# mir-group/allegro

Hardware: NVIDIA B200
Metric: atom-steps/sec (energy+forces) (higher is better)
Workload: dtype f32

## Files before the change

### allegro_b200/_lib.py

```python
from __future__ import annotations

import ctypes as C
import os
from typing import Optional, Sequence

import torch

from . import build as _build

AB2_F64, AB2_F32, AB2_BF16 = 0, 1, 2
ACT_NONE, ACT_SILU, ACT_MUL_DSILU = 0, 1, 2
EPI_NONE, EPI_MUL_DSILU = 0, 1
MAX_SEG = 4

DTYPE_ENUM = {torch.float64: AB2_F64, torch.float32: AB2_F32, torch.bfloat16: AB2_BF16}
ACC_DTYPE = {torch.float64: torch.float64, torch.float32: torch.float32, torch.bfloat16: torch.float32}

_LIB: Optional[C.CDLL] = None

_vp, _i64, _i32, _dbl = C.c_void_p, C.c_int64, C.c_int, C.c_double

_SIGNATURES = {
    "ab2_version": ([], C.c_int),
    "ab2_device_ok": ([], C.c_int),
    "ab2_last_error": ([], C.c_char_p),
    "ab2_set_option": ([C.c_char_p, _i32], C.c_int),
    "ab2_op_scatter_env": ([_i32, _i64, _i64, _dbl, _vp, _vp, _vp, _vp], C.c_int),
    "ab2_op_contract": ([_i32, _i32, _i64, _i32, _i32, _i32, _i32, _i32, _vp, _vp, _vp, _vp, _vp, _vp, _vp], C.c_int),
    "ab2_op_gather_rows": ([_i32, _i64, _i64, _dbl, _vp, _vp, _vp, _vp], C.c_int),
    "ab2_op_contract_wgrad": ([_i32, _i64, _i32, _i32, _i32, _i32, _i32, _vp, _vp, _vp, _vp, _vp, _vp, _vp], C.c_int),
    "ab2_sh_fwd": ([_i32, _i32, _i64, _vp, _vp, _vp], C.c_int),
    "ab2_sh_bwd": ([_i32, _i32, _i64, _vp, _vp, _vp, _i32, _vp], C.c_int),
    "ab2_linear": ([_i32, _i64, _i32, _i32, _i32, _vp, _vp, _vp, _vp, _vp, _i32, _vp, _vp, _i32, _vp, _vp, _vp, _vp, _i32, _vp, _i64, _vp], C.c_int),
    "ab2_linear_packed_bytes": ([_i32, _i32, _i32], C.c_int64),
    "ab2_linear_pack": ([_i32, _i32, _i32, _vp, _vp, _vp], C.c_int),
    "ab2_env_sum": ([_i32, _i32, _i64, _i32, _vp, _vp, _vp, _i64, _dbl, _vp, _vp], C.c_int),
    "ab2_env_bwd": ([_i32, _i32, _i64, _i64, _i32, _vp, _vp, _vp, _vp, _i64, _vp, _dbl, _vp, _i64, _vp, _vp], C.c_int),
    "ab2_tp_fwd": ([_i32, _i32, _i64, _i64, _i32, _i32, _i32, _i32, _vp, _vp, _vp, _vp, _vp, _vp, _i32, _vp, _vp, _i64, _vp, _vp], C.c_int),
    "ab2_tp_bwd": ([_i32, _i32, _i64, _i64, _i32, _i32, _i32, _i32, _vp, _vp, _vp, _vp, _vp, _vp, _i32, _vp, _vp, _i64, _vp, _vp, _vp, _i64, _vp, _vp, _vp], C.c_int),
    "ab2_edge_sum": ([_i32, _i64, _vp, _vp, _dbl, _vp, _vp], C.c_int),
    "ab2_edge_sum_bwd": ([_i32, _i64, _vp, _vp, _dbl, _vp, _vp], C.c_int),
    "ab2_force_scatter": ([_i32, _i64, _i64, _i64, _vp, _vp, _vp, _vp, _vp, _vp], C.c_int),
    "ab2_transpose_ui": ([_i32, _i64, _i32, _i32, _vp, _vp, _i32, _vp], C.c_int),
    "ab2_edge_vec": ([_i32, _i32, _i64, _vp, _vp, _vp, _vp, _vp, _vp], C.c_int),
    "ab2_radial_fwd": ([_i32, _i64, _i32, _i32, _dbl, _vp, _vp, _vp, _vp, _vp, _i32, _vp, _vp, _vp, _vp, _vp, _vp], C.c_int),
    "ab2_radial_pq_fwd": ([_i32, _i64, _i32, _i32, _dbl, _vp, _vp, _vp, _vp, _vp, _i32, _vp, _vp, _vp, _vp], C.c_int),
    "ab2_radial_pq_bwd": ([_i32, _i64, _i32, _i32, _dbl, _vp, _vp, _vp, _vp, _vp, _i32, _vp, _vp, _vp, _vp, _vp, _vp], C.c_int),
    "ab2_zbl": ([_i32, _i64, _i32, _dbl, _dbl, _vp, _vp, _vp, _vp, _vp, _vp, _vp, _vp, _vp], C.c_int),
    "ab2_p2p_mailbox_bytes": ([_i32, _i32], C.c_int64),
    "ab2_p2p_alloc": ([_i64, C.POINTER(C.c_void_p)], C.c_int),
    "ab2_p2p_free": ([_vp], C.c_int),
    "ab2_p2p_get_handle": ([_vp, _vp], C.c_int),
    "ab2_p2p_open_handle": ([_vp, C.POINTER(C.c_void_p)], C.c_int),
    "ab2_p2p_close_handle": ([_vp], C.c_int),
    "ab2_p2p_error": ([_vp, _i32, _i32, _vp], C.c_int),
    "ab2_p2p_begin": ([_vp, _vp], C.c_int),
    "ab2_p2p_push_rows": ([_i32, _i32, _i32, _vp, _vp, _i32, _dbl, _vp, _i32, _i32, _vp, _vp, _vp], C.c_int),
    "ab2_p2p_wait_unpack": ([_i32, _i32, _i32, _vp, _i32, _i32, _vp, _i32, _vp, _vp, _i32, _vp], C.c_int),
    "ab2_p2p_allreduce_energy": ([_vp, _i32, _i32, _i32, _vp, _vp, _vp, _vp, _vp], C.c_int),
    "ab2_nl_bin": ([_i32, _i64, _vp, _vp, _vp, _vp, _vp, _dbl, _vp, _vp], C.c_int),
    "ab2_nl_count": ([_i32, _i64, _vp, _vp, _vp, _vp, _vp, _dbl, _vp, _vp, _vp, _vp], C.c_int),
    "ab2_nl_fill": ([_i32, _i64, _vp, _vp, _vp, _vp, _vp, _dbl, _vp, _vp, _vp, _vp, _vp, _vp], C.c_int),
    "ab2_radial_bwd": ([_i32, _i64, _i32, _i32, _dbl, _vp, _vp, _vp, _vp, _vp, _i32, _vp, _vp, _vp, _vp, _vp, _vp, _vp], C.c_int),
}


def exported_symbols() -> Sequence[str]:
    return tuple(_SIGNATURES)


def lib_path() -> str:
    return _build.LIB


def load() -> C.CDLL:
    global _LIB
    if _LIB is not None:
        return _LIB
    path = lib_path()
    if not os.path.exists(path):
        if os.environ.get("ALLEGRO_B200_AUTOBUILD", "0") == "1":
            _build.build()
        else:
            raise RuntimeError(
                f"allegro_b200: CUDA extension {path} not built. Run `python -m allegro_b200.build` "
                "(or __graft_entry__.build()).  There is no CPU fallback."
            )
    lib = C.CDLL(path)
    for name, (args, res) in _SIGNATURES.items():
        fn = getattr(lib, name)
        fn.argtypes = args
        fn.restype = res
    _LIB = lib
    for kv in filter(None, os.environ.get("ALLEGRO_B200_OPTIONS", "").split(",")):
        k, v = kv.split("=")
        if lib.ab2_set_option(k.strip().encode(), int(v)) != 0:
            raise RuntimeError(f"ALLEGRO_B200_OPTIONS: unknown option {k!r}")
    return lib


class _Prof:

    def __init__(self):
        self.launches = 0
        self.enabled = False
        self.records = {}

    def reset(self):
        self.launches = 0
        self.records = {}

    def times_ms(self):
        torch.cuda.synchronize()
        return {k: [a.elapsed_time(b) for a, b in v] for k, v in self.records.items()}


PROF = _Prof()
_TAG = [""]


def set_tag(tag: str):
    _TAG[0] = tag


class _timed:
    __slots__ = ("name", "n", "ev")

    def __init__(self, name: str, n_kernels: int = 1):
        self.name, self.n = name, n_kernels

    def __enter__(self):
        PROF.launches += self.n
        if PROF.enabled:
            self.ev = (torch.cuda.Event(enable_timing=True), torch.cuda.Event(enable_timing=True))
            self.ev[0].record()
        return self

    def __exit__(self, *a):
        if PROF.enabled:
            self.ev[1].record()
            PROF.records.setdefault(self.name + "@" + _TAG[0], []).append(self.ev)
        return False


def set_option(key: str, value: int):
    _check(load().ab2_set_option(key.encode(), int(value)))


def _check(rc: int):
    if rc != 0:
        msg = load().ab2_last_error()
        raise RuntimeError(f"allegro_b200 kernel call failed (rc={rc}): {msg.decode() if msg else '?'}")


def _ptr(t: Optional[torch.Tensor]):
    if t is None:
        return None
    if not t.is_cuda:
        raise RuntimeError("allegro_b200: tensor is not on a CUDA device (no CPU fallback on the hot path)")
    return C.c_void_p(t.data_ptr())


def _stream():
    return C.c_void_p(torch.cuda.current_stream().cuda_stream)


def _contig(t: torch.Tensor, name: str):
    if not t.is_contiguous():
        raise RuntimeError(f"allegro_b200: {name} must be contiguous")
    return t


def _row_strided(t: torch.Tensor, name: str):
    if t.dim() != 2 or t.stride(1) != 1:
        raise RuntimeError(f"allegro_b200: {name} must be 2-D with unit inner stride")
    return t, int(t.stride(0))


def sh_fwd(vec: torch.Tensor, lmax: int) -> torch.Tensor:
    E = vec.shape[0]
    Y = torch.empty(E, (lmax + 1) ** 2, dtype=vec.dtype, device=vec.device)
    with _timed("sh_fwd"):
        _check(load().ab2_sh_fwd(DTYPE_ENUM[vec.dtype], lmax, E, _ptr(_contig(vec, "vec")), _ptr(Y), _stream()))
    return Y


def sh_bwd(vec: torch.Tensor, gY: torch.Tensor, lmax: int, out: Optional[torch.Tensor] = None, accumulate: bool = False):
    E = vec.shape[0]
    if out is None:
        out = torch.empty_like(vec)
        accumulate = False
    with _timed("sh_bwd"):
        _check(load().ab2_sh_bwd(DTYPE_ENUM[vec.dtype], lmax, E, _ptr(_contig(vec, "vec")), _ptr(_contig(gY, "gY")), _ptr(out), int(accumulate), _stream()))
    return out


def linear(
    a_segs: Sequence[torch.Tensor],
    W: torch.Tensor,
    o_segs: Sequence[torch.Tensor],
    o_accum: Optional[Sequence[bool]] = None,
    act: int = ACT_NONE,
    epi: int = EPI_NONE,
    aux: Optional[torch.Tensor] = None,
    W_packed: Optional[torch.Tensor] = None,
    a_aux: Optional[Sequence[Optional[torch.Tensor]]] = None,
):
    M = a_segs[0].shape[0]
    K, N = W.shape
    dt = W.dtype
    na, no = len(a_segs), len(o_segs)
    a_ptr = (C.c_void_p * na)()
    a_ld = (C.c_int64 * na)()
    a_w = (C.c_int32 * na)()
    for s, t in enumerate(a_segs):
        t, ld = _row_strided(t, f"A segment {s}")
        assert t.dtype == dt and t.shape[0] == M
        a_ptr[s], a_ld[s], a_w[s] = t.data_ptr(), ld, t.shape[1]
        _ptr(t)
    x_ptr = x_ld = None
    if a_aux is not None:
        assert act == ACT_MUL_DSILU and len(a_aux) == na
        x_ptr = (C.c_void_p * na)()
        x_ld = (C.c_int64 * na)()
        for s, t in enumerate(a_aux):
            if t is None:
                x_ptr[s], x_ld[s] = None, 0
            else:
                t, ld = _row_strided(t, f"A aux segment {s}")
                assert t.dtype == dt and t.shape == a_segs[s].shape
                x_ptr[s], x_ld[s] = t.data_ptr(), ld
                _ptr(t)
    o_ptr = (C.c_void_p * no)()
    o_ld = (C.c_int64 * no)()
    o_w = (C.c_int32 * no)()
    o_acc = (C.c_int32 * no)()
    for s, t in enumerate(o_segs):
        t, ld = _row_strided(t, f"output segment {s}")
        assert t.dtype == dt and t.shape[0] == M
        o_ptr[s], o_ld[s], o_w[s] = t.data_ptr(), ld, t.shape[1]
        o_acc[s] = int(bool(o_accum[s])) if o_accum is not None else 0
        _ptr(t)
    aux_ld = 0
    if aux is not None:
        aux, aux_ld = _row_strided(aux, "aux")
        assert aux.dtype == dt
    with _timed("linear", 1):
        _check(
            load().ab2_linear(
                DTYPE_ENUM[dt], M, K, N, na, a_ptr, a_ld, a_w, x_ptr, x_ld, act, _ptr(_contig(W, "W")), _ptr(W_packed), no, o_ptr, o_ld, o_w, o_acc, epi,
                _ptr(aux), aux_ld, _stream(),
            )
        )


def linear_pack(W: torch.Tensor) -> Optional[torch.Tensor]:
    K, N = W.shape
    nbytes = int(load().ab2_linear_packed_bytes(DTYPE_ENUM[W.dtype], K, N))
    if nbytes == 0:
        return None
    packed = torch.empty(nbytes, dtype=torch.uint8, device=W.device)
    _check(load().ab2_linear_pack(DTYPE_ENUM[W.dtype], K, N, _ptr(_contig(W, "W")), _ptr(packed), _stream()))
    return packed


def env_sum(dtype, lmax: int, N: int, U: int, row_ptr, Y, w: torch.Tensor, sf: float, out: Optional[torch.Tensor] = None):
    w, w_ld = _row_strided(w, "w")
    D = (lmax + 1) ** 2
    if out is None:
        out = torch.empty(N, D, U, dtype=ACC_DTYPE[dtype], device=Y.device)
    with _timed("env_sum"):
        _check(load().ab2_env_sum(DTYPE_ENUM[dtype], lmax, N, U, _ptr(row_ptr), _ptr(_contig(Y, "Y")), _ptr(w), w_ld, float(sf), _ptr(out), _stream()))
    return out


def env_bwd(dtype, lmax: int, U: int, ctr, Y, w: torch.Tensor, ggamma, sf: float, gw: torch.Tensor, gY: torch.Tensor, row_ptr=None):
    w, w_ld = _row_strided(w, "w")
    gw, gw_ld = _row_strided(gw, "gw")
    E = Y.shape[0]
    with _timed("env_bwd", 1):
        _check(
            load().ab2_env_bwd(
                DTYPE_ENUM[dtype], lmax, ggamma.shape[0], E, U, _ptr(row_ptr), _ptr(ctr), _ptr(_contig(Y, "Y")), _ptr(w), w_ld,
                _ptr(_contig(ggamma, "ggamma")), float(sf),
                _ptr(gw), gw_ld, _ptr(_contig(gY, "gY")), _stream(),
            )
        )


def tp_fwd(dtype, lmax, N, E, U, d_in, d_out, tab, cgw, row_ptr, ctr, gamma, Vin, Y, w0, Vout):
    implicit = Vin is None
    w0_ld = 0
    if implicit:
        w0, w0_ld = _row_strided(w0, "w0")
    with _timed("tp_fwd", 1):
        _check(
            load().ab2_tp_fwd(
                DTYPE_ENUM[dtype], lmax, N, E, U, d_in, d_out, tab.shape[0], _ptr(tab), _ptr(cgw), _ptr(row_ptr), _ptr(ctr), _ptr(gamma),
                _ptr(Vin), int(implicit), _ptr(Y), _ptr(w0) if implicit else None, w0_ld, _ptr(Vout), _stream(),
            )
        )


def tp_bwd(dtype, lmax, N, E, U, d_in, d_out, tab, cgw, row_ptr, ctr, gamma, Vin, Y, w0, gVout, gVin, gw0, gY, ggamma):
    implicit = Vin is None
    w0_ld = gw0_ld = 0
    if implicit:
        w0, w0_ld = _row_strided(w0, "w0")
        gw0, gw0_ld = _row_strided(gw0, "gw0")
    with _timed("tp_bwd", 2):
        _check(
            load().ab2_tp_bwd(
                DTYPE_ENUM[dtype], lmax, N, E, U, d_in, d_out, tab.shape[0], _ptr(tab), _ptr(cgw), _ptr(row_ptr), _ptr(ctr), _ptr(gamma),
                _ptr(Vin), int(implicit), _ptr(Y), _ptr(w0) if implicit else None, w0_ld, _ptr(gVout), _ptr(gVin),
                _ptr(gw0) if implicit else None, gw0_ld, _ptr(gY) if implicit else None, _ptr(ggamma), _stream(),
            )
        )


def edge_sum(Ez: torch.Tensor, row_ptr: torch.Tensor, factor: float) -> torch.Tensor:
    N = row_ptr.shape[0] - 1
    Ei = torch.empty(N, dtype=Ez.dtype, device=Ez.device)
    with _timed("edge_sum"):
        _check(load().ab2_edge_sum(DTYPE_ENUM[Ez.dtype], N, _ptr(row_ptr), _ptr(_contig(Ez, "Ez")), float(factor), _ptr(Ei), _stream()))
    return Ei


def edge_sum_bwd(gEi: torch.Tensor, ctr: torch.Tensor, factor: float) -> torch.Tensor:
    E = ctr.shape[0]
    gEz = torch.empty(E, dtype=gEi.dtype, device=gEi.device)
    with _timed("edge_sum_bwd"):
        _check(load().ab2_edge_sum_bwd(DTYPE_ENUM[gEi.dtype], E, _ptr(ctr), _ptr(_contig(gEi, "gEi")), float(factor), _ptr(gEz), _stream()))
    return gEz


def force_scatter(gvec: torch.Tensor, csr, num_atoms_total: int) -> torch.Tensor:
    N = csr.row_ptr.shape[0] - 1
    E = csr.nbr.shape[0]
    col_ptr, col_perm = csr.transposed(num_atoms_total)
    F = torch.empty(num_atoms_total, 3, dtype=gvec.dtype, device=gvec.device)
    with _timed("force_scatter"):
        _check(load().ab2_force_scatter(DTYPE_ENUM[gvec.dtype], N, num_atoms_total, E, _ptr(csr.row_ptr), _ptr(col_ptr), _ptr(col_perm),
                                        _ptr(_contig(gvec, "gvec")), _ptr(F), _stream()))
    return F


def transpose_ui(x: torch.Tensor, to_internal: bool) -> torch.Tensor:
    E, a, b = x.shape
    U, d = (a, b) if to_internal else (b, a)
    out = torch.empty(E, d, U, dtype=x.dtype, device=x.device) if to_internal else torch.empty(E, U, d, dtype=x.dtype, device=x.device)
    with _timed("transpose_ui"):
        _check(load().ab2_transpose_ui(DTYPE_ENUM[x.dtype], E, U, d, _ptr(_contig(x, "x")), _ptr(out), int(to_internal), _stream()))
    return out


def op_scatter_env(x2: torch.Tensor, idxs: torch.Tensor, n: int, sf: float) -> torch.Tensor:
    E = x2.shape[0]
    row = x2[0].numel() if E else 0
    gamma = torch.zeros((n,) + tuple(x2.shape[1:]), dtype=x2.dtype, device=x2.device)
    with _timed("op_scatter_env"):
        _check(load().ab2_op_scatter_env(DTYPE_ENUM[x2.dtype], E, row, float(sf), _ptr(_contig(x2, "x2")), _ptr(_contig(idxs, "idxs")), _ptr(gamma), _stream()))
    return gamma


def op_gather_rows(src: torch.Tensor, idxs: torch.Tensor, sf: float) -> torch.Tensor:
    E = idxs.shape[0]
    row = src[0].numel()
    out = torch.empty((E,) + tuple(src.shape[1:]), dtype=src.dtype, device=src.device)
    with _timed("op_gather_rows"):
        _check(load().ab2_op_gather_rows(DTYPE_ENUM[src.dtype], E, row, float(sf), _ptr(_contig(src, "src")), _ptr(_contig(idxs, "idxs")), _ptr(out), _stream()))
    return out


def op_contract(mode: int, U, d1, d2, dout, tab, cgw, a, b, idxs, out):
    E = idxs.shape[0]
    with _timed("op_contract", 1):
        _check(
            load().ab2_op_contract(
                DTYPE_ENUM[a.dtype], mode, E, U, d1, d2, dout, tab.shape[0], _ptr(tab), _ptr(cgw), _ptr(_contig(a, "a")), _ptr(_contig(b, "b")),
                _ptr(_contig(idxs, "idxs")), _ptr(out), _stream(),
            )
        )
    return out


def zbl(p_cut: float, qq: float, vec, ctr, nbr, types, Z, rmax_table, gvec: Optional[torch.Tensor]) -> torch.Tensor:
    E = ctr.shape[0]
    Ez = torch.empty(E, dtype=vec.dtype, device=vec.device)
    with _timed("zbl"):
        _check(load().ab2_zbl(DTYPE_ENUM[vec.dtype], E, Z.shape[0], float(p_cut), float(qq), _ptr(_contig(vec, "vec")), _ptr(ctr), _ptr(nbr), _ptr(types),
                              _ptr(_contig(Z, "Z")), _ptr(_contig(rmax_table, "rmax_table")), _ptr(Ez), _ptr(gvec) if gvec is not None else None, _stream()))
    return Ez


def op_contract_wgrad(U, d1, d2, dout, tab, x1, gamma, gout, idxs) -> torch.Tensor:
    E = idxs.shape[0]
    out = torch.zeros(tab.shape[0], U, dtype=x1.dtype, device=x1.device)
    with _timed("op_contract_wgrad", 1):
        _check(load().ab2_op_contract_wgrad(DTYPE_ENUM[x1.dtype], E, U, d1, d2, dout, tab.shape[0], _ptr(tab), _ptr(_contig(x1, "x1")),
                                            _ptr(_contig(gamma, "gamma")), _ptr(_contig(gout, "gout")), _ptr(_contig(idxs, "idxs")), _ptr(out), _stream()))
    return out


def edge_vec(pos: torch.Tensor, ctr, nbr, shift: Optional[torch.Tensor], acc_dtype) -> torch.Tensor:
    E = ctr.shape[0]
    vec = torch.empty(E, 3, dtype=acc_dtype, device=pos.device)
    if shift is not None:
        assert shift.dtype == pos.dtype
    with _timed("edge_vec"):
        _check(load().ab2_edge_vec(DTYPE_ENUM[pos.dtype], DTYPE_ENUM[acc_dtype], E, _ptr(_contig(pos, "pos")), _ptr(ctr), _ptr(nbr),
                                   _ptr(_contig(shift, "shift")) if shift is not None else None, _ptr(vec), _stream()))
    return vec


def radial_fwd(dtype, S_rc: int, p_cut: float, vec, ctr, nbr, types, rmax_table, bessel_w, Wb, cemb, nemb) -> torch.Tensor:
    E = ctr.shape[0]
    e0 = torch.empty(E, S_rc, dtype=dtype, device=vec.device)
    with _timed("radial_fwd"):
        _check(load().ab2_radial_fwd(DTYPE_ENUM[dtype], E, S_rc, bessel_w.numel(), float(p_cut), _ptr(vec), _ptr(ctr), _ptr(nbr), _ptr(types),
                                     _ptr(rmax_table), rmax_table.shape[0], _ptr(bessel_w), _ptr(Wb), _ptr(cemb), _ptr(nemb), _ptr(e0), _stream()))
    return e0


def radial_bwd(dtype, S_rc: int, p_cut: float, vec, ctr, nbr, types, rmax_table, bessel_w, Wb, cemb, nemb, g_e0, gvec):
    E = ctr.shape[0]
    with _timed("radial_bwd"):
        _check(load().ab2_radial_bwd(DTYPE_ENUM[dtype], E, S_rc, bessel_w.numel(), float(p_cut), _ptr(vec), _ptr(ctr), _ptr(nbr), _ptr(types),
                                     _ptr(rmax_table), rmax_table.shape[0], _ptr(bessel_w), _ptr(Wb), _ptr(cemb), _ptr(nemb),
                                     _ptr(_contig(g_e0, "g_e0")), _ptr(gvec), _stream()))


def neighbor_csr(pos: torch.Tensor, r_max: float, box, pbc=(True, True, True), origin=None, n_centres: Optional[int] = None):
    n = pos.shape[0]
    n_centres = n if n_centres is None else int(n_centres)
    box = [float(b) for b in box]
    origin = [0.0, 0.0, 0.0] if origin is None else [float(o) for o in origin]
    ncell = [max(1, int(b // float(r_max))) for b in box]
    g_box, g_org = (C.c_double * 3)(*box), (C.c_double * 3)(*origin)
    g_pbc, g_nc = (C.c_int32 * 3)(*[int(bool(p)) for p in pbc]), (C.c_int32 * 3)(*ncell)
    dt = DTYPE_ENUM[pos.dtype]
    pos = _contig(pos, "pos")
    cell_id = torch.empty(n, dtype=torch.int32, device=pos.device)
    with _timed("nl_bin"):
        _check(load().ab2_nl_bin(dt, n, _ptr(pos), g_box, g_org, g_pbc, g_nc, float(r_max), _ptr(cell_id), _stream()))
    order = torch.argsort(cell_id, stable=True).to(torch.int32)
    ncells = ncell[0] * ncell[1] * ncell[2]
    cell_start = torch.zeros(ncells + 1, dtype=torch.int32, device=pos.device)
    cell_start[1:] = torch.cumsum(torch.bincount(cell_id.long(), minlength=ncells), 0).to(torch.int32)
    counts = torch.empty(n_centres, dtype=torch.int32, device=pos.device)
    with _timed("nl_count"):
        _check(load().ab2_nl_count(dt, n_centres, _ptr(pos), g_box, g_org, g_pbc, g_nc, float(r_max), _ptr(cell_start), _ptr(order), _ptr(counts), _stream()))
    row_ptr = torch.zeros(n_centres + 1, dtype=torch.int32, device=pos.device)
    row_ptr[1:] = torch.cumsum(counts, 0).to(torch.int32)
    E = int(row_ptr[-1])
    nbr = torch.empty(E, dtype=torch.int32, device=pos.device)
    shift = torch.empty(E, 3, dtype=pos.dtype, device=pos.device)
    if E:
        with _timed("nl_fill"):
            _check(load().ab2_nl_fill(dt, n_centres, _ptr(pos), g_box, g_org, g_pbc, g_nc, float(r_max), _ptr(cell_start), _ptr(order), _ptr(row_ptr),
                                      _ptr(nbr), _ptr(shift), _stream()))
    return row_ptr, nbr, shift


def radial_pq_fwd(dtype, S: int, p_cut: float, vec, ctr, nbr, types, rmax_table, bessel_w, PQ) -> torch.Tensor:
    E = ctr.shape[0]
    out = torch.empty(E, S, dtype=dtype, device=vec.device)
    with _timed("radial_fwd"):
        _check(load().ab2_radial_pq_fwd(DTYPE_ENUM[dtype], E, S, bessel_w.numel(), float(p_cut), _ptr(vec), _ptr(ctr), _ptr(nbr), _ptr(types),
                                        _ptr(rmax_table), rmax_table.shape[0], _ptr(bessel_w), _ptr(_contig(PQ, "PQ")), _ptr(out), _stream()))
    return out


def radial_pq_bwd(dtype, S: int, p_cut: float, vec, ctr, nbr, types, rmax_table, bessel_w, PQ, g_out, aux, gvec):
    E = ctr.shape[0]
    with _timed("radial_bwd"):
        _check(load().ab2_radial_pq_bwd(DTYPE_ENUM[dtype], E, S, bessel_w.numel(), float(p_cut), _ptr(vec), _ptr(ctr), _ptr(nbr), _ptr(types),
                                        _ptr(rmax_table), rmax_table.shape[0], _ptr(bessel_w), _ptr(_contig(PQ, "PQ")), _ptr(_contig(g_out, "g_out")),
                                        _ptr(_contig(aux, "aux")) if aux is not None else None, _ptr(gvec), _stream()))
```

### allegro_b200/csrc/linear.cu

```cuda
#include "common.cuh"

struct LinSeg {
    const void* ptr;
    int64_t ld;
    int width;
    int accum;
    const void* aux;
    int64_t aux_ld;
};

struct LinParams {
    int64_t M;
    int K, N;
    int n_a;
    LinSeg a[AB2_MAX_SEG];
    int act;
    const void* W;
    int n_o;
    LinSeg o[AB2_MAX_SEG];
    int epi;
    const void* aux;
    int64_t aux_ld;
};

template <typename TAct, typename TAcc>
__device__ __forceinline__ TAcc lin_load_a(const LinParams& p, int64_t m, int k) {
#pragma unroll
    for (int s = 0; s < AB2_MAX_SEG; ++s) {
        if (s < p.n_a) {
            if (k < p.a[s].width) {
                TAcc v = to_acc<TAcc>(((const TAct*)p.a[s].ptr)[m * p.a[s].ld + k]);
                if (p.act == AB2_ACT_MUL_DSILU && p.a[s].aux)
                    v *= dsilu_f(to_acc<TAcc>(((const TAct*)p.a[s].aux)[m * p.a[s].aux_ld + k]));
                return v;
            }
            k -= p.a[s].width;
        }
    }
    return TAcc(0);
}

template <typename TAct, typename TAcc>
__global__ void __launch_bounds__(256) linear_kernel(const LinParams p) {
    constexpr int BM = 64, BN = 64, BK = 16;
    __shared__ TAcc As[BK][BM + 4];
    __shared__ TAcc Ws[BK][BN + 4];
    const int tid = threadIdx.x;
    const int tx = tid & 15, ty = tid >> 4;
    const int64_t m0 = (int64_t)blockIdx.x * BM;
    const int n0 = blockIdx.y * BN;
    TAcc acc[4][4];
#pragma unroll
    for (int i = 0; i < 4; ++i)
#pragma unroll
        for (int j = 0; j < 4; ++j) acc[i][j] = TAcc(0);

    const TAct* __restrict__ W = (const TAct*)p.W;
    for (int k0 = 0; k0 < p.K; k0 += BK) {
#pragma unroll
        for (int t = 0; t < (BM * BK) / 256; ++t) {
            const int e = tid + t * 256;
            const int kk = e & (BK - 1), r = e >> 4;
            const int64_t m = m0 + r;
            TAcc v = TAcc(0);
            if (m < p.M && k0 + kk < p.K) {
                v = lin_load_a<TAct, TAcc>(p, m, k0 + kk);
                if (p.act == AB2_ACT_SILU) v = silu_f(v);
            }
            As[kk][r] = v;
        }
#pragma unroll
        for (int t = 0; t < (BK * BN) / 256; ++t) {
            const int e = tid + t * 256;
            const int n = e & (BN - 1), kk = e >> 6;
            TAcc v = TAcc(0);
            if (k0 + kk < p.K && n0 + n < p.N) v = to_acc<TAcc>(W[(int64_t)(k0 + kk) * p.N + n0 + n]);
            Ws[kk][n] = v;
        }
        __syncthreads();
#pragma unroll
        for (int kk = 0; kk < BK; ++kk) {
            TAcc a[4], b[4];
#pragma unroll
            for (int i = 0; i < 4; ++i) a[i] = As[kk][ty * 4 + i];
#pragma unroll
            for (int j = 0; j < 4; ++j) b[j] = Ws[kk][tx * 4 + j];
#pragma unroll
            for (int i = 0; i < 4; ++i)
#pragma unroll
                for (int j = 0; j < 4; ++j) acc[i][j] += a[i] * b[j];
        }
        __syncthreads();
    }

#pragma unroll
    for (int i = 0; i < 4; ++i) {
        const int64_t m = m0 + ty * 4 + i;
        if (m >= p.M) continue;
#pragma unroll
        for (int j = 0; j < 4; ++j) {
            int n = n0 + tx * 4 + j;
            if (n >= p.N) continue;
            TAcc v = acc[i][j];
            if (p.epi == AB2_EPI_MUL_DSILU) v *= dsilu_f(to_acc<TAcc>(((const TAct*)p.aux)[m * p.aux_ld + n]));
#pragma unroll
            for (int s = 0; s < AB2_MAX_SEG; ++s) {
                if (s < p.n_o) {
                    if (n >= 0 && n < p.o[s].width) {
                        TAct* dst = (TAct*)p.o[s].ptr + m * p.o[s].ld + n;
                        if (p.o[s].accum) v += to_acc<TAcc>(*dst);
                        *dst = from_acc<TAct>(v);
                        n = -1 << 20;
                    }
                    n -= p.o[s].width;
                }
            }
        }
    }
}

int ab2_linear_tc_try(int dtype, int64_t M, int K, int N, int n_a, const void* const* a_ptr, const int64_t* a_ld,
                      const int32_t* a_width, const void* const* a_aux, const int64_t* a_aux_ld, int act, const void* Wpacked, int n_o, void* const* o_ptr, const int64_t* o_ld,
                      const int32_t* o_width, const int32_t* o_accum, int epi, const void* aux, int64_t aux_ld, cudaStream_t st);

extern "C" int ab2_linear(int dtype, int64_t M, int K, int N, int n_a, const void* const* a_ptr, const int64_t* a_ld,
                          const int32_t* a_width, const void* const* a_aux, const int64_t* a_aux_ld, int act, const void* W,
                          const void* Wpacked, int n_o, void* const* o_ptr,
                          const int64_t* o_ld, const int32_t* o_width, const int32_t* o_accum, int epi, const void* aux,
                          int64_t aux_ld, void* stream) {
    if (M == 0) return 0;
    AB2_CHECK_ARG(n_a >= 1 && n_a <= AB2_MAX_SEG && n_o >= 1 && n_o <= AB2_MAX_SEG, "segment count");
    AB2_CHECK_ARG(K > 0 && N > 0 && W, "shape");
    AB2_CHECK_ARG(epi == AB2_EPI_NONE || aux, "aux required for dsilu epilogue");
    LinParams p;
    memset(&p, 0, sizeof(p));
    p.M = M; p.K = K; p.N = N; p.n_a = n_a; p.act = act; p.W = W; p.n_o = n_o; p.epi = epi; p.aux = aux; p.aux_ld = aux_ld;
    int ks = 0, ns = 0;
    for (int s = 0; s < n_a; ++s) {
        AB2_CHECK_ARG(a_ptr[s] && a_width[s] > 0 && a_ld[s] >= a_width[s], "A segment");
        p.a[s].ptr = a_ptr[s]; p.a[s].ld = a_ld[s]; p.a[s].width = a_width[s]; ks += a_width[s];
        p.a[s].aux = a_aux ? a_aux[s] : nullptr;
        p.a[s].aux_ld = (a_aux && a_aux_ld) ? a_aux_ld[s] : 0;
    }
    for (int s = 0; s < n_o; ++s) {
        AB2_CHECK_ARG(o_ptr[s] && o_width[s] > 0 && o_ld[s] >= o_width[s], "output segment");
        p.o[s].ptr = o_ptr[s]; p.o[s].ld = o_ld[s]; p.o[s].width = o_width[s]; p.o[s].accum = o_accum ? o_accum[s] : 0;
        ns += o_width[s];
    }
    AB2_CHECK_ARG(ks == K, "A segment widths must sum to K");
    AB2_CHECK_ARG(ns == N, "output segment widths must sum to N");
    cudaStream_t st = (cudaStream_t)stream;
    const int tc = Wpacked ? ab2_linear_tc_try(dtype, M, K, N, n_a, a_ptr, a_ld, a_width, a_aux, a_aux_ld, act, Wpacked, n_o, o_ptr, o_ld, o_width,
                                               o_accum, epi, aux, aux_ld, st)
                           : -1;
    if (tc == 0) {
        AB2_CUDA_LAUNCH_CHECK();
        return 0;
    }
    if (tc > 0) {
        ab2_set_error("%s:%d: tensor-core linear: a column slice failed to launch (K=%d, N=%d)", __FILE__, __LINE__, K, N);
        return 2;
    }
    dim3 grid(ab2_blocks(M, 64), (unsigned)((N + 63) / 64));
    AB2_DISPATCH_DTYPE(dtype, linear_kernel<TAct, TAcc><<<grid, 256, 0, st>>>(p));
    AB2_CUDA_LAUNCH_CHECK();
    return 0;
}
```

### allegro_b200/csrc/linear_tc.cu

```cuda
#include <cuda.h>

#include "common.cuh"

extern int g_ab2_opt_linear_tc;
extern int g_ab2_opt_linear_tma;
extern int g_ab2_opt_tc_debug;

namespace {

constexpr int BM = 128;
constexpr int KC = 32;
constexpr int NSTAGE = 4;
constexpr int RAW_DEPTH = 4;
constexpr int RAW_STAGE = 256 * 4 * 16;
constexpr int EPI_LD = 36;
constexpr int EPI_BYTES = 4 * 32 * EPI_LD * 4;
constexpr int PF_BYTES = 2 * EPI_BYTES;
constexpr int STAGE_HALF = BM * KC * 2;
constexpr int NPROD = 8;
constexpr int NTHREADS = (NPROD + 1 + 4) * 32;
constexpr int MAX_W_BYTES = 128 * 1024;
constexpr int MAX_K = 512;
constexpr int MAX_CHUNK = 8;
constexpr int TAIL_BARS = 96, TAIL_SLOT = 16, TAIL_CHUNK = MAX_CHUNK * 32, TAIL_KMAP = (MAX_K / 8) * 16;
constexpr int TAIL_BYTES = TAIL_BARS + TAIL_SLOT + TAIL_CHUNK + 2 * TAIL_KMAP;

struct TcSeg {
    const void* ptr;
    int64_t ld;
    int width;
    int accum;
    const void* aux;
    int64_t aux_ld;
};

struct TcParams {
    int64_t M;
    int K, N, Npad;
    int n_a;
    TcSeg a[AB2_MAX_SEG];
    int act;
    const void* Wpacked;
    const void* Wlo;
    int n_o;
    TcSeg o[AB2_MAX_SEG];
    int epi;
    const void* aux;
    int64_t aux_ld;
    int64_t num_tiles;
    int nstage;
    int debug;
    int pf_mode;
    int raw_depth;
    int has_aux;
};

struct KEnt {
    const void* ptr;
    int64_t ld;
};
struct ChunkInfo {
    float* optr;
    const float* aptr;
    int64_t ld;
    int32_t accum;
    int32_t ok;
};
static_assert(sizeof(KEnt) == 16 && sizeof(ChunkInfo) == 32, "table entry sizes");

__device__ __forceinline__ uint32_t smem_u32(const void* p) { return (uint32_t)__cvta_generic_to_shared(p); }

__device__ __forceinline__ void mbar_init(uint32_t bar, uint32_t count) {
    asm volatile("mbarrier.init.shared::cta.b64 [%0], %1;" ::"r"(bar), "r"(count));
}
__device__ __forceinline__ void mbar_arrive(uint32_t bar) {
    asm volatile("mbarrier.arrive.shared::cta.b64 _, [%0];" ::"r"(bar) : "memory");
}
__device__ __forceinline__ void mbar_arrive_relaxed(uint32_t bar) {
    asm volatile("mbarrier.arrive.relaxed.cta.shared::cta.b64 _, [%0];" ::"r"(bar));
}
__device__ __forceinline__ void mbar_wait(uint32_t bar, uint32_t parity) {
    asm volatile(
        "{\n\t"
        ".reg .pred p;\n\t"
        "WAIT_LOOP:\n\t"
        "mbarrier.try_wait.parity.shared::cta.b64 p, [%0], %1;\n\t"
        "@p bra WAIT_DONE;\n\t"
        "bra WAIT_LOOP;\n\t"
        "WAIT_DONE:\n\t"
        "}" ::"r"(bar),
        "r"(parity)
        : "memory");
}
__device__ __forceinline__ void fence_proxy_async() { asm volatile("fence.proxy.async.shared::cta;" ::: "memory"); }
__device__ __forceinline__ void fence_barrier_init() { asm volatile("fence.mbarrier_init.release.cluster;" ::: "memory"); }
__device__ __forceinline__ void tc_fence_before() { asm volatile("tcgen05.fence::before_thread_sync;" ::: "memory"); }
__device__ __forceinline__ void tc_fence_after() { asm volatile("tcgen05.fence::after_thread_sync;" ::: "memory"); }

__device__ __forceinline__ void tmem_alloc(uint32_t dst_smem, uint32_t ncols) {
    asm volatile("tcgen05.alloc.cta_group::1.sync.aligned.shared::cta.b32 [%0], %1;" ::"r"(dst_smem), "r"(ncols) : "memory");
    asm volatile("tcgen05.relinquish_alloc_permit.cta_group::1.sync.aligned;" ::: "memory");
}
__device__ __forceinline__ void tmem_dealloc(uint32_t taddr, uint32_t ncols) {
    asm volatile("tcgen05.dealloc.cta_group::1.sync.aligned.b32 %0, %1;" ::"r"(taddr), "r"(ncols) : "memory");
}
__device__ __forceinline__ void umma_commit(uint32_t bar) {
    asm volatile("tcgen05.commit.cta_group::1.mbarrier::arrive::one.shared::cluster.b64 [%0];" ::"r"(bar) : "memory");
}
__device__ __forceinline__ void umma_bf16(uint32_t d_tmem, uint64_t adesc, uint64_t bdesc, uint32_t idesc, uint32_t accumulate) {
    asm volatile(
        "{\n\t"
        ".reg .pred p;\n\t"
        "setp.ne.b32 p, %4, 0;\n\t"
        "tcgen05.mma.cta_group::1.kind::f16 [%0], %1, %2, %3, p;\n\t"
        "}" ::"r"(d_tmem),
        "l"(adesc), "l"(bdesc), "r"(idesc), "r"(accumulate)
        : "memory");
}
__device__ __forceinline__ void tmem_ld16_nowait(uint32_t taddr, uint32_t (&r)[16]) {
    asm volatile(
        "tcgen05.ld.sync.aligned.32x32b.x16.b32 {%0,%1,%2,%3,%4,%5,%6,%7,%8,%9,%10,%11,%12,%13,%14,%15}, [%16];"
        : "=r"(r[0]), "=r"(r[1]), "=r"(r[2]), "=r"(r[3]), "=r"(r[4]), "=r"(r[5]), "=r"(r[6]), "=r"(r[7]), "=r"(r[8]), "=r"(r[9]),
          "=r"(r[10]), "=r"(r[11]), "=r"(r[12]), "=r"(r[13]), "=r"(r[14]), "=r"(r[15])
        : "r"(taddr)
        : "memory");
}
__device__ __forceinline__ void tmem_ld_wait() { asm volatile("tcgen05.wait::ld.sync.aligned;" ::: "memory"); }
__device__ __forceinline__ void tmem_ld16(uint32_t taddr, uint32_t (&r)[16]) {
    asm volatile(
        "tcgen05.ld.sync.aligned.32x32b.x16.b32 {%0,%1,%2,%3,%4,%5,%6,%7,%8,%9,%10,%11,%12,%13,%14,%15}, [%16];"
        : "=r"(r[0]), "=r"(r[1]), "=r"(r[2]), "=r"(r[3]), "=r"(r[4]), "=r"(r[5]), "=r"(r[6]), "=r"(r[7]), "=r"(r[8]), "=r"(r[9]),
          "=r"(r[10]), "=r"(r[11]), "=r"(r[12]), "=r"(r[13]), "=r"(r[14]), "=r"(r[15])
        : "r"(taddr)
        : "memory");
    asm volatile("tcgen05.wait::ld.sync.aligned;" ::: "memory");
}

__device__ __forceinline__ void cp_async16(uint32_t dst_smem, const void* src, uint32_t src_bytes) {
    asm volatile("cp.async.cg.shared.global [%0], [%1], 16, %2;" ::"r"(dst_smem), "l"(src), "r"(src_bytes) : "memory");
}
__device__ __forceinline__ void cp_async_commit() { asm volatile("cp.async.commit_group;" ::: "memory"); }
template <int N>
__device__ __forceinline__ void cp_async_wait() { asm volatile("cp.async.wait_group %0;" ::"n"(N) : "memory"); }

__device__ __forceinline__ void stg128(float* p, const float4& v) {
    asm volatile("st.global.v4.f32 [%0], {%1, %2, %3, %4};" ::"l"(p), "f"(v.x), "f"(v.y), "f"(v.z), "f"(v.w) : "memory");
}
__device__ __forceinline__ float4 ldg128(const float* p) {
    float4 v;
    asm volatile("ld.global.v4.f32 {%0, %1, %2, %3}, [%4];" : "=f"(v.x), "=f"(v.y), "=f"(v.z), "=f"(v.w) : "l"(p));
    return v;
}
__device__ __forceinline__ float4 ldg128_nc(const float* p) {
    float4 v;
    asm volatile("ld.global.nc.v4.f32 {%0, %1, %2, %3}, [%4];" : "=f"(v.x), "=f"(v.y), "=f"(v.z), "=f"(v.w) : "l"(p));
    return v;
}

template <typename TSrc>
__device__ __forceinline__ const TSrc* seg_ptr(const TcParams& p, int64_t m, int k) {
#pragma unroll
    for (int s = 0; s < AB2_MAX_SEG; ++s) {
        if (s < p.n_a) {
            if (k < p.a[s].width) return (const TSrc*)p.a[s].ptr + m * p.a[s].ld + k;
            k -= p.a[s].width;
        }
    }
    return nullptr;
}

template <typename TSrc>
__device__ __forceinline__ const TSrc* seg_aux_ptr(const TcParams& p, int64_t m, int k) {
#pragma unroll
    for (int s = 0; s < AB2_MAX_SEG; ++s) {
        if (s < p.n_a) {
            if (k < p.a[s].width) return p.a[s].aux ? (const TSrc*)p.a[s].aux + m * p.a[s].aux_ld + k : nullptr;
            k -= p.a[s].width;
        }
    }
    return nullptr;
}

__device__ __forceinline__ uint64_t make_desc(uint32_t saddr, uint32_t lbo_bytes, uint32_t sbo_bytes) {
    uint64_t d = 0;
    d |= (uint64_t)((saddr >> 4) & 0x3FFF);
    d |= (uint64_t)((lbo_bytes >> 4) & 0x3FFF) << 16;
    d |= (uint64_t)((sbo_bytes >> 4) & 0x3FFF) << 32;
    d |= (uint64_t)1 << 46;
    return d;
}

__device__ __forceinline__ float sigmoid_fast(float x) { return __fdividef(1.f, 1.f + __expf(-x)); }
__device__ __forceinline__ float silu_fast(float x) { return x * sigmoid_fast(x); }
__device__ __forceinline__ float dsilu_fast(float x) {
    const float sg = sigmoid_fast(x);
    return sg * (1.f + x * (1.f - sg));
}

__device__ __forceinline__ uint32_t pack_bf16x2(float a, float b) {
    __nv_bfloat162 v = __floats2bfloat162_rn(a, b);
    return *reinterpret_cast<uint32_t*>(&v);
}

template <typename TSrc>
__device__ __forceinline__ void load8(const TcParams& p, int64_t m, int k, float (&v)[8]) {
#pragma unroll
    for (int s = 0; s < AB2_MAX_SEG; ++s) {
        if (s < p.n_a) {
            if (k < p.a[s].width) {
                if constexpr (sizeof(TSrc) == 4) {
                    const float4* src = reinterpret_cast<const float4*>((const float*)p.a[s].ptr + m * p.a[s].ld + k);
                    const float4 x = __ldg(src), y = __ldg(src + 1);
                    v[0] = x.x; v[1] = x.y; v[2] = x.z; v[3] = x.w; v[4] = y.x; v[5] = y.y; v[6] = y.z; v[7] = y.w;
                } else {
                    const uint4 x = __ldg(reinterpret_cast<const uint4*>((const bf16*)p.a[s].ptr + m * p.a[s].ld + k));
                    const __nv_bfloat162* h = reinterpret_cast<const __nv_bfloat162*>(&x);
#pragma unroll
                    for (int t = 0; t < 4; ++t) {
                        const float2 f = __bfloat1622float2(h[t]);
                        v[2 * t] = f.x; v[2 * t + 1] = f.y;
                    }
                }
                return;
            }
            k -= p.a[s].width;
        }
    }
#pragma unroll
    for (int t = 0; t < 8; ++t) v[t] = 0.f;
}


template <typename TSrc>
__device__ __forceinline__ ChunkInfo tc_chunk_info(const TcParams& p, int c0) {
    ChunkInfo info{nullptr, nullptr, 0, 0, 0};
    if (sizeof(TSrc) == 4 && c0 + 32 <= p.N && !(p.debug & 64)) {
        int lo = 0, seg = -1, seg_lo = 0;
#pragma unroll
        for (int s2 = 0; s2 < AB2_MAX_SEG; ++s2) {
            if (s2 < p.n_o) {
                if (c0 >= lo && c0 + 32 <= lo + p.o[s2].width) { seg = s2; seg_lo = lo; }
                lo += p.o[s2].width;
            }
        }
        if (seg >= 0) {
            float* base = (float*)p.o[seg].ptr + (c0 - seg_lo);
            bool ok = !(reinterpret_cast<uintptr_t>(base) & 15) && !((p.o[seg].ld * 4) & 15);
            if (p.epi == AB2_EPI_MUL_DSILU &&
                ((reinterpret_cast<uintptr_t>((const float*)p.aux + c0) & 15) || ((p.aux_ld * 4) & 15))) ok = false;
            info.optr = base;
            info.aptr = (const float*)p.aux + c0;
            info.ld = p.o[seg].ld;
            info.accum = p.o[seg].accum;
            info.ok = ok ? 1 : 0;
        }
    }
    return info;
}

struct TcCtx {
    uint8_t* sW;
    uint8_t* sA;
    float* sEpi;
    float* sPf;
    ChunkInfo* sChunk;
    uint32_t bar0;
    uint32_t tmem_base;
    int nkb, stage_bytes, w_half;
    uint32_t idesc;
    __device__ __forceinline__ uint32_t full_bar(int s) const { return bar0 + 8u * s; }
    __device__ __forceinline__ uint32_t empty_bar(int s) const { return bar0 + 8u * (NSTAGE + s); }
    __device__ __forceinline__ uint32_t tfull_bar(int a) const { return bar0 + 8u * (2 * NSTAGE + a); }
    __device__ __forceinline__ uint32_t tempty_bar(int a) const { return bar0 + 8u * (2 * NSTAGE + 2 + a); }
};

template <bool SPLIT>
__device__ __forceinline__ void tc_mma_role(const TcParams& p, const TcCtx& c, int lane) {
    const int nkb = c.nkb, stage_bytes = c.stage_bytes, w_half = c.w_half;
    const uint32_t tmem_base = c.tmem_base, idesc = c.idesc;
    uint8_t* sW = c.sW;
    uint8_t* sA = c.sA;
    auto full_bar = [&](int s) { return c.full_bar(s); };
    auto empty_bar = [&](int s) { return c.empty_bar(s); };
    auto tfull_bar = [&](int a) { return c.tfull_bar(a); };
    auto tempty_bar = [&](int a) { return c.tempty_bar(a); };
    int stage = 0;
    uint32_t phase = 0;
    int64_t it = 0;
    const uint32_t sW_u = smem_u32(sW);
    const uint32_t w_sbo = (uint32_t)(p.K / 8) * 128;
    for (int64_t tile = blockIdx.x; tile < p.num_tiles; tile += gridDim.x, ++it) {
        const int a = (int)(it & 1);
        const uint32_t aphase = (uint32_t)((it >> 1) & 1);
        mbar_wait(tempty_bar(a), aphase ^ 1);
        tc_fence_after();
        const uint32_t d_tmem = tmem_base + (uint32_t)(a * 256);
        for (int kb = 0; kb < nkb; ++kb) {
            mbar_wait(full_bar(stage), phase);
            tc_fence_after();
            if (lane == 0) {
                const uint32_t a_hi = smem_u32(sA + stage * stage_bytes);
                const int ksteps = min(2, (p.K - kb * KC) / 16);
                for (int ks = 0; ks < ((p.debug & 4) ? 0 : ksteps); ++ks) {
                    const uint64_t da_hi = make_desc(a_hi + ks * 256, 128, (KC / 8) * 128);
                    const uint32_t wk = sW_u + (uint32_t)(kb * (KC / 8) + ks * 2) * 128;
                    const uint64_t db_hi = make_desc(wk, 128, w_sbo);
                    umma_bf16(d_tmem, da_hi, db_hi, idesc, (kb | ks) ? 1u : 0u);
                    if constexpr (SPLIT) {
                        const uint64_t da_lo = make_desc(a_hi + STAGE_HALF + ks * 256, 128, (KC / 8) * 128);
                        const uint64_t db_lo = make_desc(wk + w_half, 128, w_sbo);
                        umma_bf16(d_tmem, da_lo, db_hi, idesc, 1u);
                        umma_bf16(d_tmem, da_hi, db_lo, idesc, 1u);
                    }
                }
                umma_commit(empty_bar(stage));
                if (kb == nkb - 1) umma_commit(tfull_bar(a));
            }
            __syncwarp();
            if (++stage == p.nstage) { stage = 0; phase ^= 1; }
        }
    }
}

template <typename TSrc, int PF>
__device__ __forceinline__ void tc_epilogue_role(const TcParams& p, const TcCtx& c, int warp, int lane) {
    const uint32_t tmem_base = c.tmem_base;
    float* sEpi = c.sEpi;
    float* sPf = c.sPf;
    ChunkInfo* sChunk = c.sChunk;
    auto tfull_bar = [&](int a) { return c.tfull_bar(a); };
    auto tempty_bar = [&](int a) { return c.tempty_bar(a); };
    const int q = warp & 3;
    int64_t it = 0;
    for (int64_t tile = blockIdx.x; tile < p.num_tiles; tile += gridDim.x, ++it) {
        const int a = (int)(it & 1);
        const uint32_t aphase = (uint32_t)((it >> 1) & 1);
        const int64_t m_base = tile * BM + q * 32;
        const int64_t left64 = p.M - m_base;
        const int rows_left = left64 >= 32 ? 32 : (left64 > 0 ? (int)left64 : 0);
        const bool full = rows_left == 32;
        const int rsub = lane >> 3, c4 = lane & 7;
        auto row_of = [&](int itr) { const int r = itr * 4 + rsub; return full ? r : (r < rows_left ? r : rows_left - 1); };
        float* pfw = sPf + q * 2 * 32 * EPI_LD;
        auto prefetch = [&](int c0) {
            if constexpr (PF == 0) return;
            if (c0 < p.Npad && rows_left > 0) {
                const ChunkInfo ci = sChunk[c0 >> 5];
                if (ci.ok && (PF == 1 || ci.accum)) {
                    const int64_t gld = (PF == 1) ? p.aux_ld : ci.ld;
                    const float* tb = ((PF == 1) ? ci.aptr : (const float*)ci.optr) + m_base * gld + c4 * 4;
                    const uint32_t gl = (uint32_t)gld;
                    float* dstb = pfw + ((c0 >> 5) & 1) * 32 * EPI_LD + c4 * 4;
#pragma unroll
                    for (int itr = 0; itr < 8; ++itr)
                        cp_async16(smem_u32(dstb + (itr * 4 + rsub) * EPI_LD), tb + (uint32_t)row_of(itr) * gl, 16u);
                }
            }
            cp_async_commit();
        };
        prefetch(0);
        prefetch(32);
        mbar_wait(tfull_bar(a), aphase);
        tc_fence_after();
        const int64_t m = tile * BM + q * 32 + lane;
        const uint32_t t_row = tmem_base + ((uint32_t)(q * 32) << 16) + (uint32_t)(a * 256);
        auto process = [&](int c0, const uint32_t (&r)[16]) {
            if (m >= p.M) return;
            float v[16];
#pragma unroll
            for (int j = 0; j < 16; ++j) v[j] = __uint_as_float(r[j]);
            if (p.epi == AB2_EPI_MUL_DSILU) {
                const TSrc* ax = (const TSrc*)p.aux + m * p.aux_ld + c0;
                if (sizeof(TSrc) == 4 && c0 + 16 <= p.N && ((reinterpret_cast<uintptr_t>(ax) & 15) == 0)) {
                    const float4* a4 = reinterpret_cast<const float4*>(ax);
#pragma unroll
                    for (int t = 0; t < 4; ++t) {
                        const float4 x = __ldg(a4 + t);
                        v[4 * t] *= dsilu_f(x.x); v[4 * t + 1] *= dsilu_f(x.y); v[4 * t + 2] *= dsilu_f(x.z); v[4 * t + 3] *= dsilu_f(x.w);
                    }
                } else {
#pragma unroll
                    for (int j = 0; j < 16; ++j)
                        if (c0 + j < p.N) v[j] *= dsilu_f(to_acc<float>(ax[j]));
                }
            }
            int seg_lo = 0;
#pragma unroll
            for (int s = 0; s < AB2_MAX_SEG; ++s) {
                if (s < p.n_o) {
                    const int seg_hi = seg_lo + p.o[s].width;
                    const int lo = max(seg_lo, c0), hi = min(seg_hi, min(c0 + 16, p.N));
                    if (lo < hi) {
                        TSrc* dst = (TSrc*)p.o[s].ptr + m * p.o[s].ld + (lo - seg_lo);
                        const bool vec = (sizeof(TSrc) == 4) && (hi - lo == 16) && ((reinterpret_cast<uintptr_t>(dst) & 15) == 0);
                        if (vec) {
                            float4* d4 = reinterpret_cast<float4*>(dst);
#pragma unroll
                            for (int t = 0; t < 4; ++t) {
                                float4 o4 = make_float4(v[4 * t], v[4 * t + 1], v[4 * t + 2], v[4 * t + 3]);
                                if (p.o[s].accum) {
                                    const float4 old = d4[t];
                                    o4.x += old.x; o4.y += old.y; o4.z += old.z; o4.w += old.w;
                                }
                                d4[t] = o4;
                            }
                        } else {
#pragma unroll
                            for (int j = 0; j < 16; ++j) {
                                const int n = c0 + j;
                                if (n >= lo && n < hi) {
                                    float x = v[j];
                                    if (p.o[s].accum) x += to_acc<float>(dst[n - lo]);
                                    dst[n - lo] = from_acc<TSrc>(x);
                                }
                            }
                        }
                    }
                    seg_lo = seg_hi;
                }
            }
        };
        float* stg = sEpi + q * 32 * EPI_LD;
        for (int c0 = 0; c0 < p.Npad; c0 += 32) {
            uint32_t r0[16], r1[16];
            const bool two = c0 + 16 < p.Npad;
            tmem_ld16_nowait(t_row + c0, r0);
            if (two) tmem_ld16_nowait(t_row + c0 + 16, r1);
            tmem_ld_wait();
            const ChunkInfo ci = sChunk[c0 >> 5];
            if constexpr (PF != 0) cp_async_wait<1>();
            if ((p.debug & 1) || rows_left == 0) {
            } else if (ci.ok) {
                float4* srow = reinterpret_cast<float4*>(stg + lane * EPI_LD);
#pragma unroll
                for (int t = 0; t < 4; ++t) {
                    srow[t] = make_float4(__uint_as_float(r0[4 * t]), __uint_as_float(r0[4 * t + 1]), __uint_as_float(r0[4 * t + 2]), __uint_as_float(r0[4 * t + 3]));
                    srow[4 + t] = make_float4(__uint_as_float(r1[4 * t]), __uint_as_float(r1[4 * t + 1]), __uint_as_float(r1[4 * t + 2]), __uint_as_float(r1[4 * t + 3]));
                }
                __syncwarp();
                float4 x[8];
#pragma unroll
                for (int itr = 0; itr < 8; ++itr) x[itr] = *reinterpret_cast<const float4*>(stg + (itr * 4 + rsub) * EPI_LD + c4 * 4);
                float* tb = ci.optr + m_base * ci.ld + c4 * 4;
                const uint32_t ol = (uint32_t)ci.ld;
                uint32_t off[8];
#pragma unroll
                for (int itr = 0; itr < 8; ++itr) off[itr] = (uint32_t)row_of(itr) * ol;
                const float* pfb = pfw + ((c0 >> 5) & 1) * 32 * EPI_LD;
                if (p.epi == AB2_EPI_MUL_DSILU) {
                    float4 ax[8];
                    const float* ab = ci.aptr + m_base * p.aux_ld + c4 * 4;
                    const uint32_t al = (uint32_t)p.aux_ld;
#pragma unroll
                    for (int itr = 0; itr < 8; ++itr)
                        ax[itr] = (PF == 1) ? *reinterpret_cast<const float4*>(pfb + (itr * 4 + rsub) * EPI_LD + c4 * 4)
                                                   : ldg128_nc(ab + (uint32_t)row_of(itr) * al);
#pragma unroll
                    for (int itr = 0; itr < 8; ++itr) {
                        x[itr].x *= dsilu_fast(ax[itr].x); x[itr].y *= dsilu_fast(ax[itr].y);
                        x[itr].z *= dsilu_fast(ax[itr].z); x[itr].w *= dsilu_fast(ax[itr].w);
                    }
                }
                if (ci.accum) {
                    float4 old[8];
#pragma unroll
                    for (int itr = 0; itr < 8; ++itr)
                        old[itr] = (PF == 2) ? *reinterpret_cast<const float4*>(pfb + (itr * 4 + rsub) * EPI_LD + c4 * 4)
                                                    : ldg128(tb + off[itr]);
#pragma unroll
                    for (int itr = 0; itr < 8; ++itr) {
                        x[itr].x += old[itr].x; x[itr].y += old[itr].y; x[itr].z += old[itr].z; x[itr].w += old[itr].w;
                    }
                }
                if (full) {
#pragma unroll
                    for (int itr = 0; itr < 8; ++itr) stg128(tb + off[itr], x[itr]);
                } else {
#pragma unroll
                    for (int itr = 0; itr < 8; ++itr)
                        if (itr * 4 + rsub < rows_left) stg128(tb + off[itr], x[itr]);
                }
                __syncwarp();
            } else {
                process(c0, r0);
                if (two) process(c0 + 16, r1);
            }
            if constexpr (PF != 0) {
                __syncwarp();
                prefetch(c0 + 64);
            }
        }
        tc_fence_before();
        if (p.debug & 8) mbar_arrive(tempty_bar(a));
        else mbar_arrive_relaxed(tempty_bar(a));
    }
}

template <typename TSrc, bool SPLIT, int PF>
__global__ void __launch_bounds__(NTHREADS, 1) linear_tc_kernel(const TcParams p) {
    extern __shared__ __align__(1024) uint8_t smem[];
    const int warp = threadIdx.x >> 5, lane = threadIdx.x & 31;
    const int w_half = p.Npad * p.K * 2;
    const int w_bytes = SPLIT ? 2 * w_half : w_half;
    uint8_t* sW = smem;
    uint8_t* sA = smem + ((w_bytes + 127) & ~127);
    const int stage_bytes = SPLIT ? 2 * STAGE_HALF : STAGE_HALF;
    uint8_t* sRaw = sA + p.nstage * stage_bytes;
    const int raw_stage = RAW_STAGE * (p.has_aux ? 2 : 1);
    float* sEpi = reinterpret_cast<float*>(sRaw + p.raw_depth * raw_stage);
    float* sPf = reinterpret_cast<float*>(reinterpret_cast<uint8_t*>(sEpi) + EPI_BYTES);
    uint64_t* bars = reinterpret_cast<uint64_t*>(reinterpret_cast<uint8_t*>(sEpi) + EPI_BYTES + (PF ? PF_BYTES : 0));
    uint32_t* tmem_slot = reinterpret_cast<uint32_t*>(bars + 2 * NSTAGE + 4);
    static_assert((2 * NSTAGE + 4) * 8 == TAIL_BARS, "barrier block size");
    ChunkInfo* sChunk = reinterpret_cast<ChunkInfo*>(reinterpret_cast<uint8_t*>(bars) + TAIL_BARS + TAIL_SLOT);
    KEnt* sKmap = reinterpret_cast<KEnt*>(reinterpret_cast<uint8_t*>(sChunk) + TAIL_CHUNK);
    KEnt* sKaux = sKmap + MAX_K / 8;
    const uint32_t bar0 = smem_u32(bars);
    auto full_bar = [&](int s) { return bar0 + 8u * s; };
    auto empty_bar = [&](int s) { return bar0 + 8u * (NSTAGE + s); };
    auto tfull_bar = [&](int a) { return bar0 + 8u * (2 * NSTAGE + a); };
    auto tempty_bar = [&](int a) { return bar0 + 8u * (2 * NSTAGE + 2 + a); };

    if (threadIdx.x == 0) {
        for (int s = 0; s < NSTAGE; ++s) {
            mbar_init(full_bar(s), NPROD * 32);
            mbar_init(empty_bar(s), 1);
        }
        for (int a = 0; a < 2; ++a) {
            mbar_init(tfull_bar(a), 1);
            mbar_init(tempty_bar(a), 128);
        }
        fence_barrier_init();
    }
    if (warp == NPROD) tmem_alloc(smem_u32(tmem_slot), 512);
    if (threadIdx.x < MAX_K / 8) {
        const int e = threadIdx.x;
        KEnt ent{nullptr, 0}, aent{nullptr, 0};
        int kk = e * 8;
        bool found = kk >= p.K;
#pragma unroll
        for (int sgi = 0; sgi < AB2_MAX_SEG; ++sgi) {
            if (sgi < p.n_a && !found) {
                if (kk < p.a[sgi].width) {
                    ent.ptr = (const TSrc*)p.a[sgi].ptr + kk;
                    ent.ld = p.a[sgi].ld;
                    if (p.a[sgi].aux) {
                        aent.ptr = (const TSrc*)p.a[sgi].aux + kk;
                        aent.ld = p.a[sgi].aux_ld;
                    }
                    found = true;
                }
                kk -= p.a[sgi].width;
            }
        }
        sKmap[e] = ent;
        sKaux[e] = aent;
    } else if (threadIdx.x < MAX_K / 8 + MAX_CHUNK) {
        sChunk[threadIdx.x - MAX_K / 8] = tc_chunk_info<TSrc>(p, (threadIdx.x - MAX_K / 8) * 32);
    }
    {
        const uint4* src = reinterpret_cast<const uint4*>(p.Wpacked);
        uint4* dst = reinterpret_cast<uint4*>(sW);
        for (int e = threadIdx.x; e < w_half / 16; e += NTHREADS) dst[e] = __ldg(src + e);
        if constexpr (SPLIT) {
            const uint4* srcl = reinterpret_cast<const uint4*>(p.Wlo);
            uint4* dstl = reinterpret_cast<uint4*>(sW + w_half);
            for (int e = threadIdx.x; e < w_half / 16; e += NTHREADS) dstl[e] = __ldg(srcl + e);
        }
    }
    fence_proxy_async();
    tc_fence_before();
    __syncthreads();
    tc_fence_after();
    const uint32_t tmem_base = *tmem_slot;

    const int nkb = (p.K + KC - 1) / KC;
    const uint32_t idesc = (1u << 4) | (1u << 7) | (1u << 10) | ((uint32_t)(p.Npad >> 3) << 17) | ((uint32_t)(BM >> 4) << 24);
    TcCtx ctx;
    ctx.sW = sW; ctx.sA = sA; ctx.sEpi = sEpi; ctx.sPf = sPf; ctx.sChunk = sChunk; ctx.bar0 = bar0; ctx.tmem_base = tmem_base;
    ctx.nkb = nkb; ctx.stage_bytes = stage_bytes; ctx.w_half = w_half; ctx.idesc = idesc;

    if (warp < NPROD) {
        constexpr int GPW = 16 / NPROD;
        const int r8 = lane & 7, kc = lane >> 3;
        const int64_t my_tiles = (p.num_tiles > blockIdx.x) ? (p.num_tiles - blockIdx.x + gridDim.x - 1) / gridDim.x : 0;
        const int64_t total = my_tiles * nkb;
        int stage = 0;
        uint32_t phase = 0;
        constexpr int CH = (sizeof(TSrc) == 4) ? 2 : 1;
        const uint32_t raw_u = smem_u32(sRaw);
        int64_t i_tile = blockIdx.x, i_seq = 0;
        int i_kb = 0, i_slot = 0, f_kb = 0, f_slot = 0;
        auto issue = [&]() {
            if (i_seq < total) {
                const int64_t row0 = i_tile * BM;
                const int64_t left = p.M - row0;
                const int rows_left = left < BM ? (int)left : BM;
                const KEnt e = sKmap[i_kb * (KC / 8) + kc];
                const bool kok = e.ptr != nullptr && !(p.debug & 2);
                const uint8_t* tb = reinterpret_cast<const uint8_t*>(e.ptr) + row0 * e.ld * (int64_t)sizeof(TSrc);
                const uint32_t pitch = (uint32_t)e.ld * (uint32_t)sizeof(TSrc);
                KEnt ea{nullptr, 0};
                if (p.has_aux) ea = sKaux[i_kb * (KC / 8) + kc];
                const uint8_t* tba = reinterpret_cast<const uint8_t*>(ea.ptr) + row0 * ea.ld * (int64_t)sizeof(TSrc);
                const uint32_t pitch_a = (uint32_t)ea.ld * (uint32_t)sizeof(TSrc);
#pragma unroll
                for (int i = 0; i < GPW; ++i) {
                    const int row = (warp * GPW + i) * 8 + r8;
                    const bool inb = kok && row < rows_left;
                    const uint8_t* src = tb + (uint32_t)row * pitch;
#pragma unroll
                    for (int h = 0; h < CH; ++h) {
                        const uint32_t dst = raw_u + (uint32_t)(i_slot * raw_stage + ((i * CH + h) * 256 + threadIdx.x) * 16);
                        cp_async16(dst, inb ? (const void*)(src + 16 * h) : p.Wpacked, inb ? 16u : 0u);
                    }
                    if (p.has_aux) {
                        const bool ain = inb && ea.ptr != nullptr;
                        const uint8_t* ax = tba + (uint32_t)row * pitch_a;
#pragma unroll
                        for (int h = 0; h < CH; ++h) {
                            const uint32_t dst = raw_u + (uint32_t)(i_slot * raw_stage + ((4 + i * CH + h) * 256 + threadIdx.x) * 16);
                            cp_async16(dst, ain ? (const void*)(ax + 16 * h) : p.Wpacked, ain ? 16u : 0u);
                        }
                    }
                }
            }
            cp_async_commit();
            ++i_seq;
            if (++i_slot == p.raw_depth) i_slot = 0;
            if (++i_kb == nkb) { i_kb = 0; i_tile += gridDim.x; }
        };
        auto fetch = [&](float (&v)[GPW][8]) {
            const uint8_t* base = sRaw + f_slot * raw_stage;
            auto rd8 = [&](int chunk0, float (&o)[8]) {
                if constexpr (sizeof(TSrc) == 4) {
                    const float4 x = *reinterpret_cast<const float4*>(base + ((chunk0 + 0) * 256 + threadIdx.x) * 16);
                    const float4 y = *reinterpret_cast<const float4*>(base + ((chunk0 + 1) * 256 + threadIdx.x) * 16);
                    o[0] = x.x; o[1] = x.y; o[2] = x.z; o[3] = x.w; o[4] = y.x; o[5] = y.y; o[6] = y.z; o[7] = y.w;
                } else {
                    const uint4 x = *reinterpret_cast<const uint4*>(base + (chunk0 * 256 + threadIdx.x) * 16);
                    const __nv_bfloat162* hh = reinterpret_cast<const __nv_bfloat162*>(&x);
#pragma unroll
                    for (int t = 0; t < 4; ++t) {
                        const float2 f = __bfloat1622float2(hh[t]);
                        o[2 * t] = f.x; o[2 * t + 1] = f.y;
                    }
                }
            };
            const bool has = p.has_aux && sKaux[f_kb * (KC / 8) + kc].ptr != nullptr;
#pragma unroll
            for (int i = 0; i < GPW; ++i) {
                rd8(i * CH, v[i]);
                if (p.has_aux) {
                    float w[8];
                    rd8(4 + i * CH, w);
                    if (has) {
#pragma unroll
                        for (int t = 0; t < 8; ++t) v[i][t] *= dsilu_fast(w[t]);
                    }
                }
            }
            if (++f_slot == p.raw_depth) f_slot = 0;
            if (++f_kb == nkb) f_kb = 0;
        };
        auto emit = [&](float (&v)[GPW][8]) {
            mbar_wait(empty_bar(stage), phase ^ 1);
            uint8_t* st_hi = sA + stage * stage_bytes;
#pragma unroll
            for (int i = 0; i < GPW; ++i) {
                if (p.act == AB2_ACT_SILU) {
#pragma unroll
                    for (int t = 0; t < 8; ++t) v[i][t] = silu_fast(v[i][t]);
                }
                const int g = warp * GPW + i;
                const uint32_t off = g * (KC / 8) * 128 + kc * 128 + r8 * 16;
                uint32_t hi[4];
                float lo[8];
#pragma unroll
                for (int t = 0; t < 4; ++t) {
                    const __nv_bfloat16 h0 = __float2bfloat16_rn(v[i][2 * t]), h1 = __float2bfloat16_rn(v[i][2 * t + 1]);
                    lo[2 * t] = v[i][2 * t] - __bfloat162float(h0);
                    lo[2 * t + 1] = v[i][2 * t + 1] - __bfloat162float(h1);
                    __nv_bfloat162 hh;
                    hh.x = h0; hh.y = h1;
                    hi[t] = *reinterpret_cast<uint32_t*>(&hh);
                }
                *reinterpret_cast<uint4*>(st_hi + off) = make_uint4(hi[0], hi[1], hi[2], hi[3]);
                if constexpr (SPLIT) {
                    *reinterpret_cast<uint4*>(st_hi + STAGE_HALF + off) =
                        make_uint4(pack_bf16x2(lo[0], lo[1]), pack_bf16x2(lo[2], lo[3]), pack_bf16x2(lo[4], lo[5]), pack_bf16x2(lo[6], lo[7]));
                }
            }
            fence_proxy_async();
            mbar_arrive(full_bar(stage));
            if (++stage == p.nstage) { stage = 0; phase ^= 1; }
        };
        static_assert(GPW == 2, "raw slot layout assumes 2 row groups per producer warp");
        for (int d = 0; d < p.raw_depth; ++d) issue();
        for (int64_t seq = 0; seq < total; ++seq) {
            if (p.raw_depth == 4) cp_async_wait<3>();
            else cp_async_wait<1>();
            float v[GPW][8];
            fetch(v);
            issue();
            emit(v);
        }
        cp_async_wait<0>();
    } else if (warp == NPROD) {
        tc_mma_role<SPLIT>(p, ctx, lane);
    } else {
        tc_epilogue_role<TSrc, PF>(p, ctx, warp, lane);
    }
    tc_fence_before();
    __syncthreads();
    if (warp == NPROD) tmem_dealloc(tmem_base, 512);
}

constexpr int TMA_THREADS = NTHREADS + 32;
constexpr int TMA_BOX_BYTES = BM * KC * 4;

struct alignas(64) TmaMaps {
    CUtensorMap a[AB2_MAX_SEG];
    CUtensorMap x[AB2_MAX_SEG];
};

__device__ __forceinline__ void tma_load_2d(uint32_t dst, const CUtensorMap* map, int x, int y, uint32_t bar) {
    asm volatile("cp.async.bulk.tensor.2d.shared::cluster.global.mbarrier::complete_tx::bytes [%0], [%1, {%3, %4}], [%2];" ::"r"(dst),
                 "l"(reinterpret_cast<uint64_t>(map)), "r"(bar), "r"(x), "r"(y)
                 : "memory");
}
__device__ __forceinline__ void mbar_expect_tx(uint32_t bar, uint32_t bytes) {
    asm volatile("mbarrier.arrive.expect_tx.shared::cta.b64 _, [%0], %1;" ::"r"(bar), "r"(bytes) : "memory");
}

template <int PF, int G>
__global__ void __launch_bounds__(TMA_THREADS, 1) linear_tma_kernel(const TcParams p, const __grid_constant__ TmaMaps maps, int NR) {
    constexpr int WPG = NPROD / G;
    constexpr int RGW = 16 / WPG;
    using TSrc = float;
    constexpr bool SPLIT = true;
    extern __shared__ __align__(1024) uint8_t smem[];
    const int warp = threadIdx.x >> 5, lane = threadIdx.x & 31;
    const int w_half = p.Npad * p.K * 2;
    const int w_bytes = 2 * w_half;
    const int stage_bytes = 2 * STAGE_HALF;
    const int raw_slot = TMA_BOX_BYTES * (p.has_aux ? 2 : 1);
    uint8_t* sRaw = smem + ((1024u - (smem_u32(smem) & 1023u)) & 1023u);
    uint8_t* sW = sRaw + (size_t)NR * raw_slot;
    uint8_t* sA = sW + ((w_bytes + 127) & ~127);
    float* sEpi = reinterpret_cast<float*>(sA + p.nstage * stage_bytes);
    float* sPf = reinterpret_cast<float*>(reinterpret_cast<uint8_t*>(sEpi) + EPI_BYTES);
    uint64_t* bars = reinterpret_cast<uint64_t*>(reinterpret_cast<uint8_t*>(sEpi) + EPI_BYTES + (PF ? PF_BYTES : 0));
    uint32_t* tmem_slot = reinterpret_cast<uint32_t*>(bars + 2 * NSTAGE + 4);
    ChunkInfo* sChunk = reinterpret_cast<ChunkInfo*>(reinterpret_cast<uint8_t*>(bars) + TAIL_BARS + TAIL_SLOT);
    int4* sKseg = reinterpret_cast<int4*>(reinterpret_cast<uint8_t*>(sChunk) + TAIL_CHUNK);
    uint64_t* rbars = reinterpret_cast<uint64_t*>(reinterpret_cast<uint8_t*>(sKseg) + (MAX_K / 32) * 16);
    const uint32_t bar0 = smem_u32(bars), rbar0 = smem_u32(rbars);
    auto rfull_bar = [&](int s) { return rbar0 + 8u * s; };
    auto rempty_bar = [&](int s) { return rbar0 + 8u * (8 + s); };
    const int nkb = p.K / KC;

    if (threadIdx.x == 0) {
        for (int s = 0; s < NSTAGE; ++s) {
            mbar_init(bar0 + 8u * s, WPG * 32);
            mbar_init(bar0 + 8u * (NSTAGE + s), 1);
        }
        for (int a = 0; a < 2; ++a) {
            mbar_init(bar0 + 8u * (2 * NSTAGE + a), 1);
            mbar_init(bar0 + 8u * (2 * NSTAGE + 2 + a), 128);
        }
        for (int s = 0; s < 8; ++s) {
            mbar_init(rfull_bar(s), 1);
            mbar_init(rempty_bar(s), WPG * 32);
        }
        fence_barrier_init();
    }
    if (warp == NPROD) tmem_alloc(smem_u32(tmem_slot), 512);
    if (threadIdx.x < MAX_K / 32) {
        int kk = threadIdx.x * KC;
        int4 ent = make_int4(-1, 0, 0, 0);
#pragma unroll
        for (int sgi = 0; sgi < AB2_MAX_SEG; ++sgi) {
            if (sgi < p.n_a && ent.x < 0 && kk < p.K) {
                if (kk < p.a[sgi].width) ent = make_int4(sgi, kk, p.a[sgi].aux ? 1 : 0, 0);
                kk -= p.a[sgi].width;
            }
        }
        sKseg[threadIdx.x] = ent;
    } else if (threadIdx.x >= 64 && threadIdx.x < 64 + MAX_CHUNK) {
        sChunk[threadIdx.x - 64] = tc_chunk_info<TSrc>(p, (threadIdx.x - 64) * 32);
    }
    {
        const uint4* src = reinterpret_cast<const uint4*>(p.Wpacked);
        uint4* dst = reinterpret_cast<uint4*>(sW);
        for (int e = threadIdx.x; e < w_half / 16; e += TMA_THREADS) dst[e] = __ldg(src + e);
        const uint4* srcl = reinterpret_cast<const uint4*>(p.Wlo);
        uint4* dstl = reinterpret_cast<uint4*>(sW + w_half);
        for (int e = threadIdx.x; e < w_half / 16; e += TMA_THREADS) dstl[e] = __ldg(srcl + e);
    }
    fence_proxy_async();
    tc_fence_before();
    __syncthreads();
    tc_fence_after();
    TcCtx ctx;
    ctx.sW = sW; ctx.sA = sA; ctx.sEpi = sEpi; ctx.sPf = sPf; ctx.sChunk = sChunk; ctx.bar0 = bar0; ctx.tmem_base = *tmem_slot;
    ctx.nkb = nkb; ctx.stage_bytes = stage_bytes; ctx.w_half = w_half;
    ctx.idesc = (1u << 4) | (1u << 7) | (1u << 10) | ((uint32_t)(p.Npad >> 3) << 17) | ((uint32_t)(BM >> 4) << 24);
    const int64_t my_tiles = (p.num_tiles > blockIdx.x) ? (p.num_tiles - blockIdx.x + gridDim.x - 1) / gridDim.x : 0;
    const int64_t total = my_tiles * nkb;

    if (warp == NPROD + 5) {
        if (lane == 0) {
            for (int sgi = 0; sgi < p.n_a; ++sgi) {
                asm volatile("prefetch.tensormap [%0];" ::"l"(reinterpret_cast<uint64_t>(&maps.a[sgi])) : "memory");
                if (p.a[sgi].aux) asm volatile("prefetch.tensormap [%0];" ::"l"(reinterpret_cast<uint64_t>(&maps.x[sgi])) : "memory");
            }
            int rs = 0, kb = 0;
            uint32_t rph = 0;
            int64_t tile = blockIdx.x;
            for (int64_t qs = 0; qs < total; ++qs) {
                mbar_wait(rempty_bar(rs), rph ^ 1);
                const int4 ent = sKseg[kb];
                const uint32_t dst = smem_u32(sRaw + (size_t)rs * raw_slot);
                const bool ax = p.has_aux && ent.z;
                mbar_expect_tx(rfull_bar(rs), TMA_BOX_BYTES * (ax ? 2u : 1u));
                if (!(p.debug & 2)) {
                    tma_load_2d(dst, &maps.a[ent.x], ent.y, (int)(tile * BM), rfull_bar(rs));
                    if (ax) tma_load_2d(dst + TMA_BOX_BYTES, &maps.x[ent.x], ent.y, (int)(tile * BM), rfull_bar(rs));
                } else {
                    asm volatile("mbarrier.complete_tx.shared::cta.b64 [%0], %1;" ::"r"(rfull_bar(rs)), "r"(TMA_BOX_BYTES * (ax ? 2u : 1u)) : "memory");
                }
                if (++rs == NR) { rs = 0; rph ^= 1; }
                if (++kb == nkb) { kb = 0; tile += gridDim.x; }
            }
        }
    } else if (warp < NPROD) {
        const int grp = warp / WPG, sub = warp % WPG;
        const int r8 = lane & 7, kc = lane >> 3;
        int rs = grp % NR, cs = grp % p.nstage, kb = grp % nkb;
        uint32_t rph = (uint32_t)((grp / NR) & 1), cph = (uint32_t)((grp / p.nstage) & 1);
        for (int64_t qs = grp; qs < total; qs += G) {
            mbar_wait(rfull_bar(rs), rph);
            const uint8_t* raw = sRaw + (size_t)rs * raw_slot;
            const bool ax = p.has_aux && sKseg[kb].z;
            float v[RGW][8];
#pragma unroll
            for (int i = 0; i < RGW; ++i) {
                const int row = (sub * RGW + i) * 8 + r8;
                const uint8_t* rp = raw + row * 128;
                const float4 x = *reinterpret_cast<const float4*>(rp + (((2 * kc) ^ r8) << 4));
                const float4 y = *reinterpret_cast<const float4*>(rp + (((2 * kc + 1) ^ r8) << 4));
                v[i][0] = x.x; v[i][1] = x.y; v[i][2] = x.z; v[i][3] = x.w; v[i][4] = y.x; v[i][5] = y.y; v[i][6] = y.z; v[i][7] = y.w;
            }
            if (ax) {
#pragma unroll
                for (int i = 0; i < RGW; ++i) {
                    const int row = (sub * RGW + i) * 8 + r8;
                    const uint8_t* rp = raw + TMA_BOX_BYTES + row * 128;
                    const float4 x = *reinterpret_cast<const float4*>(rp + (((2 * kc) ^ r8) << 4));
                    const float4 y = *reinterpret_cast<const float4*>(rp + (((2 * kc + 1) ^ r8) << 4));
                    v[i][0] *= dsilu_fast(x.x); v[i][1] *= dsilu_fast(x.y); v[i][2] *= dsilu_fast(x.z); v[i][3] *= dsilu_fast(x.w);
                    v[i][4] *= dsilu_fast(y.x); v[i][5] *= dsilu_fast(y.y); v[i][6] *= dsilu_fast(y.z); v[i][7] *= dsilu_fast(y.w);
                }
            }
            __syncwarp();
            mbar_arrive(rempty_bar(rs));
            mbar_wait(ctx.empty_bar(cs), cph ^ 1);
            uint8_t* st_hi = sA + cs * stage_bytes;
#pragma unroll
            for (int i = 0; i < RGW; ++i) {
                if (p.act == AB2_ACT_SILU) {
#pragma unroll
                    for (int t = 0; t < 8; ++t) v[i][t] = silu_fast(v[i][t]);
                }
                const int g = sub * RGW + i;
                const uint32_t off = g * (KC / 8) * 128 + kc * 128 + r8 * 16;
                uint32_t hi[4];
                float lo[8];
#pragma unroll
                for (int t = 0; t < 4; ++t) {
                    const __nv_bfloat16 h0 = __float2bfloat16_rn(v[i][2 * t]), h1 = __float2bfloat16_rn(v[i][2 * t + 1]);
                    lo[2 * t] = v[i][2 * t] - __bfloat162float(h0);
                    lo[2 * t + 1] = v[i][2 * t + 1] - __bfloat162float(h1);
                    __nv_bfloat162 hh;
                    hh.x = h0; hh.y = h1;
                    hi[t] = *reinterpret_cast<uint32_t*>(&hh);
                }
                *reinterpret_cast<uint4*>(st_hi + off) = make_uint4(hi[0], hi[1], hi[2], hi[3]);
                *reinterpret_cast<uint4*>(st_hi + STAGE_HALF + off) =
                    make_uint4(pack_bf16x2(lo[0], lo[1]), pack_bf16x2(lo[2], lo[3]), pack_bf16x2(lo[4], lo[5]), pack_bf16x2(lo[6], lo[7]));
            }
            fence_proxy_async();
            mbar_arrive(ctx.full_bar(cs));
            rs += G; if (rs >= NR) { rs -= NR; rph ^= 1; }
            cs += G; if (cs >= p.nstage) { cs -= p.nstage; cph ^= 1; }
            kb += G; while (kb >= nkb) kb -= nkb;
        }
    } else if (warp == NPROD) {
        tc_mma_role<SPLIT>(p, ctx, lane);
    } else {
        tc_epilogue_role<TSrc, PF>(p, ctx, warp, lane);
    }
    tc_fence_before();
    __syncthreads();
    if (warp == NPROD) tmem_dealloc(ctx.tmem_base, 512);
}

template <typename TSrc>
__global__ void pack_w_kernel(int K, int N, int Npad, const TSrc* __restrict__ W, bf16* __restrict__ out) {
    const int e = blockIdx.x * blockDim.x + threadIdx.x;
    if (e >= Npad * K) return;
    const int n = e / K, k = e % K;
    const float w = (n < N) ? to_acc<float>(W[(int64_t)k * N + n]) : 0.f;
    const bf16 h = __float2bfloat16_rn(w);
    const bf16 l = __float2bfloat16_rn(w - __bfloat162float(h));
    const int64_t off = ((int64_t)(n / 8) * (K / 8) + k / 8) * 64 + (n % 8) * 8 + (k % 8);
    out[off] = h;
    out[(int64_t)Npad * K + off] = l;
}

}

static int tc_npad(int N) { return (N + 15) / 16 * 16; }

extern "C" int64_t ab2_linear_packed_bytes(int dtype, int K, int N) {
    if (dtype == AB2_F64 || K % 16 != 0 || K <= 0 || K > MAX_K || N <= 0) return 0;
    const int Npad = tc_npad(N);
    return (int64_t)Npad * K * 2 * 2;
}

static int tc_slice_cap(int dtype, int K) {
    const int per_col = K * 2 * (dtype == AB2_F32 ? 2 : 1);
    int cap = (MAX_W_BYTES / per_col) / 32 * 32;
    if (cap > 256) cap = 256;
    return cap;
}

extern "C" int ab2_linear_pack(int dtype, int K, int N, const void* W, void* packed, void* stream) {
    AB2_CHECK_ARG(ab2_linear_packed_bytes(dtype, K, N) > 0, "shape not supported by the tensor-core path");
    AB2_CHECK_ARG(W && packed, "null pointer");
    const int Npad = tc_npad(N);
    cudaStream_t st = (cudaStream_t)stream;
    const int total = Npad * K;
    if (dtype == AB2_F32)
        pack_w_kernel<float><<<(total + 255) / 256, 256, 0, st>>>(K, N, Npad, (const float*)W, (bf16*)packed);
    else
        pack_w_kernel<bf16><<<(total + 255) / 256, 256, 0, st>>>(K, N, Npad, (const bf16*)W, (bf16*)packed);
    AB2_CUDA_LAUNCH_CHECK();
    return 0;
}

typedef CUresult (*EncodeTiledFn)(CUtensorMap*, CUtensorMapDataType, cuuint32_t, void*, const cuuint64_t*, const cuuint64_t*, const cuuint32_t*,
                                  const cuuint32_t*, CUtensorMapInterleave, CUtensorMapSwizzle, CUtensorMapL2promotion, CUtensorMapFloatOOBfill);

static EncodeTiledFn tc_encode_fn() {
    static EncodeTiledFn fn = nullptr;
    static bool tried = false;
    if (!tried) {
        tried = true;
        void* ptr = nullptr;
        cudaDriverEntryPointQueryResult qres;
        if (cudaGetDriverEntryPoint("cuTensorMapEncodeTiled", &ptr, cudaEnableDefault, &qres) == cudaSuccess && qres == cudaDriverEntryPointSuccess)
            fn = reinterpret_cast<EncodeTiledFn>(ptr);
        else
            cudaGetLastError();
    }
    return fn;
}

static bool tc_make_map(CUtensorMap* map, const void* ptr, int64_t ld, int width, int64_t M) {
    EncodeTiledFn fn = tc_encode_fn();
    if (!fn) return false;
    const cuuint64_t dims[2] = {(cuuint64_t)width, (cuuint64_t)M};
    const cuuint64_t strides[1] = {(cuuint64_t)ld * 4};
    const cuuint32_t box[2] = {(cuuint32_t)KC, (cuuint32_t)BM};
    const cuuint32_t estr[2] = {1, 1};
    return fn(map, CU_TENSOR_MAP_DATA_TYPE_FLOAT32, 2, const_cast<void*>(ptr), dims, strides, box, estr, CU_TENSOR_MAP_INTERLEAVE_NONE,
              CU_TENSOR_MAP_SWIZZLE_128B, CU_TENSOR_MAP_L2_PROMOTION_L2_128B, CU_TENSOR_MAP_FLOAT_OOB_FILL_NONE) == CUDA_SUCCESS;
}

static int tc_launch_tma(TcParams& p, int pf_mode, int w_bytes, int stage_bytes, int max_smem, unsigned grid, cudaStream_t st, bool dry) {
    TmaMaps maps;
    memset(&maps, 0, sizeof(maps));
    if (!tc_encode_fn()) return -1;
    for (int s = 0; s < p.n_a && !dry; ++s) {
        if (!tc_make_map(&maps.a[s], p.a[s].ptr, p.a[s].ld, p.a[s].width, p.M)) return -1;
        if (p.a[s].aux && !tc_make_map(&maps.x[s], p.a[s].aux, p.a[s].aux_ld, p.a[s].width, p.M)) return -1;
    }
    const int raw_slot = TMA_BOX_BYTES * (p.has_aux ? 2 : 1);
    const int plans[6][3] = {{4, 8, 4}, {4, 4, 4}, {2, 4, 4}, {2, 2, 4}, {2, 4, 2}, {2, 2, 2}};
    int G = 0, NR = 0, nstage = 0;
    size_t smem = 0;
    for (int q = 0; q < 6 && !G; ++q) {
        const size_t need = 1024 + ((w_bytes + 127) & ~127) + (size_t)plans[q][2] * stage_bytes + EPI_BYTES + (pf_mode ? PF_BYTES : 0) + TAIL_BYTES +
                            (size_t)plans[q][1] * raw_slot;
        if (need <= (size_t)max_smem) { G = plans[q][0]; NR = plans[q][1]; nstage = plans[q][2]; smem = need; }
    }
    if (!G) return -1;
    if (dry) return 0;
    p.nstage = nstage;
    auto go = [&](auto kern) -> int {
        if (cudaFuncSetAttribute(kern, cudaFuncAttributeMaxDynamicSharedMemorySize, (int)smem) != cudaSuccess) {
            cudaGetLastError();
            return -1;
        }
        kern<<<grid, TMA_THREADS, smem, st>>>(p, maps, NR);
        return 0;
    };
    if (G == 4) {
        if (pf_mode == 1) return go(linear_tma_kernel<1, 4>);
        if (pf_mode == 2) return go(linear_tma_kernel<2, 4>);
        return go(linear_tma_kernel<0, 4>);
    }
    if (pf_mode == 1) return go(linear_tma_kernel<1, 2>);
    if (pf_mode == 2) return go(linear_tma_kernel<2, 2>);
    return go(linear_tma_kernel<0, 2>);
}

static int tc_launch_slice(int dtype, int64_t M, int K, int N, int n_a, const void* const* a_ptr, const int64_t* a_ld,
                           const int32_t* a_width, const void* const* a_aux, const int64_t* a_aux_ld, int act, const void* Whi, const void* Wlo,
                           int n_o, void* const* o_ptr, const int64_t* o_ld, const int32_t* o_width, const int32_t* o_accum, int epi,
                           const void* aux, int64_t aux_ld, cudaStream_t st, bool dry = false) {
    const int has_aux = (act == AB2_ACT_MUL_DSILU && a_aux) ? 1 : 0;
    int pf_mode = 0;
    if (dtype == AB2_F32) {
        if (epi == AB2_EPI_MUL_DSILU) pf_mode = 1;
        else if (o_accum) for (int s = 0; s < n_o; ++s) if (o_accum[s]) pf_mode = 2;
    }
    static int num_sms = 0;
    static int max_smem = 0;
    if (num_sms == 0) {
        int dev = 0;
        cudaGetDevice(&dev);
        cudaDeviceGetAttribute(&num_sms, cudaDevAttrMultiProcessorCount, dev);
        cudaDeviceGetAttribute(&max_smem, cudaDevAttrMaxSharedMemoryPerBlockOptin, dev);
    }
    TcParams p;
    memset(&p, 0, sizeof(p));
    p.M = M; p.K = K; p.N = N; p.Npad = tc_npad(N); p.n_a = n_a; p.act = act; p.Wpacked = Whi; p.Wlo = Wlo; p.n_o = n_o;
    p.epi = epi; p.aux = aux; p.aux_ld = aux_ld; p.num_tiles = (M + BM - 1) / BM;
    for (int s = 0; s < n_a; ++s) {
        p.a[s].ptr = a_ptr[s]; p.a[s].ld = a_ld[s]; p.a[s].width = a_width[s];
        p.a[s].aux = has_aux ? a_aux[s] : nullptr; p.a[s].aux_ld = has_aux ? a_aux_ld[s] : 0;
    }
    p.has_aux = has_aux;
    for (int s = 0; s < n_o; ++s) { p.o[s].ptr = o_ptr[s]; p.o[s].ld = o_ld[s]; p.o[s].width = o_width[s]; p.o[s].accum = o_accum ? o_accum[s] : 0; }
    const bool split = dtype == AB2_F32;
    const int w_bytes = p.Npad * K * 2 * (split ? 2 : 1);
    const int stage_bytes = STAGE_HALF * (split ? 2 : 1);
    int nstage = 0, raw_depth = 0;
    size_t smem = 0;
    const int raw_stage = RAW_STAGE * (has_aux ? 2 : 1);
    const int plans[4][2] = {{4, NSTAGE}, {4, 2}, {2, NSTAGE}, {2, 2}};
    for (int q = 0; q < 4 && !nstage; ++q) {
        const size_t need = ((w_bytes + 127) & ~127) + (size_t)plans[q][1] * stage_bytes + (size_t)plans[q][0] * raw_stage + EPI_BYTES +
                            (pf_mode ? PF_BYTES : 0) + TAIL_BYTES;
        if ((int)need <= max_smem) { raw_depth = plans[q][0]; nstage = plans[q][1]; smem = need; }
    }
    if (!nstage) return -1;
    if (dry) return 0;
    p.nstage = nstage;
    p.raw_depth = raw_depth;
    p.pf_mode = pf_mode;
    p.debug = g_ab2_opt_tc_debug;
    const unsigned grid = (unsigned)((p.num_tiles < num_sms) ? p.num_tiles : num_sms);
    bool tma_ok = g_ab2_opt_linear_tma && split && K % KC == 0 && M < ((int64_t)1 << 31);
    for (int s = 0; s < n_a && tma_ok; ++s) tma_ok = a_width[s] % KC == 0;
    if (tma_ok) {
        const int rc = tc_launch_tma(p, pf_mode, w_bytes, stage_bytes, max_smem, grid, st, dry);
        if (rc == 0) return 0;
    }
    auto go = [&](auto kern) -> int {
        if (cudaFuncSetAttribute(kern, cudaFuncAttributeMaxDynamicSharedMemorySize, (int)smem) != cudaSuccess) {
            cudaGetLastError();
            return -1;
        }
        kern<<<grid, NTHREADS, smem, st>>>(p);
        return 0;
    };
    if (split) {
        if (pf_mode == 1) return go(linear_tc_kernel<float, true, 1>);
        if (pf_mode == 2) return go(linear_tc_kernel<float, true, 2>);
        return go(linear_tc_kernel<float, true, 0>);
    }
    return go(linear_tc_kernel<bf16, false, 0>);
}

int ab2_linear_tc_try(int dtype, int64_t M, int K, int N, int n_a, const void* const* a_ptr, const int64_t* a_ld,
                      const int32_t* a_width, const void* const* a_aux, const int64_t* a_aux_ld, int act, const void* Wpacked, int n_o, void* const* o_ptr, const int64_t* o_ld,
                      const int32_t* o_width, const int32_t* o_accum, int epi, const void* aux, int64_t aux_ld, cudaStream_t st) {
    if (!g_ab2_opt_linear_tc || !Wpacked || dtype == AB2_F64) return -1;
    if (ab2_linear_packed_bytes(dtype, K, N) == 0) return -1;
    const int esz = (dtype == AB2_F32) ? 4 : 2;
    for (int s = 0; s < n_a; ++s) {
        if (a_width[s] % 8 != 0) return -1;
        if ((reinterpret_cast<uintptr_t>(a_ptr[s]) % 16) != 0 || (a_ld[s] * esz) % 16 != 0) return -1;
        if (act == AB2_ACT_MUL_DSILU && a_aux && a_aux[s] &&
            ((reinterpret_cast<uintptr_t>(a_aux[s]) % 16) != 0 || (a_aux_ld[s] * esz) % 16 != 0)) return -1;
    }
    const int cap = tc_slice_cap(dtype, K);
    if (cap < 32) return -1;
    const int Npad_full = tc_npad(N);
    const int nslices = (N + cap - 1) / cap;
    int width = ((N + nslices - 1) / nslices + 31) / 32 * 32;
    if (width > cap) width = cap;
    int32_t any_accum = 0;
    for (int s = 0; s < n_o && o_accum; ++s) any_accum |= o_accum[s];
    while (true) {
        const int probe = width < N ? width : N;
        if (tc_launch_slice(dtype, M, K, probe, n_a, a_ptr, a_ld, a_width, a_aux, a_aux_ld, act, Wpacked, Wpacked, 1, o_ptr, o_ld, &probe, &any_accum, epi,
                            aux, aux_ld, st, true) == 0)
            break;
        if (width <= 32) return -1;
        width = (width / 2 + 31) / 32 * 32;
    }
    const uint8_t* hi = reinterpret_cast<const uint8_t*>(Wpacked);
    const uint8_t* lo = hi + (size_t)Npad_full * K * 2;
    for (int n0 = 0; n0 < N; n0 += width) {
        const int ns = (N - n0 < width) ? (N - n0) : width;
        void* so_ptr[AB2_MAX_SEG];
        int64_t so_ld[AB2_MAX_SEG];
        int32_t so_w[AB2_MAX_SEG], so_acc[AB2_MAX_SEG];
        int cnt = 0, seg_lo = 0;
        for (int s = 0; s < n_o; ++s) {
            const int seg_hi = seg_lo + o_width[s];
            const int a = n0 > seg_lo ? n0 : seg_lo, b = (n0 + ns) < seg_hi ? (n0 + ns) : seg_hi;
            if (a < b) {
                so_ptr[cnt] = reinterpret_cast<uint8_t*>(o_ptr[s]) + (size_t)(a - seg_lo) * esz;
                so_ld[cnt] = o_ld[s];
                so_w[cnt] = b - a;
                so_acc[cnt] = o_accum ? o_accum[s] : 0;
                ++cnt;
            }
            seg_lo = seg_hi;
        }
        const void* aux_s = aux ? reinterpret_cast<const uint8_t*>(aux) + (size_t)n0 * esz : nullptr;
        const int rc = tc_launch_slice(dtype, M, K, ns, n_a, a_ptr, a_ld, a_width, a_aux, a_aux_ld, act, hi + (size_t)n0 * K * 2,
                                       lo + (size_t)n0 * K * 2, cnt, so_ptr, so_ld, so_w, so_acc, epi, aux_s, aux_ld, st);
        if (rc != 0) return n0 == 0 ? -1 : 1;
    }
    return 0;
}
```

### allegro_b200/nn/_mlp.py

```python
from __future__ import annotations

import math
from typing import List, Optional, Sequence

import torch

from .. import _lib

def _silu_gain() -> float:
    n = 200001
    z = torch.linspace(-12.0, 12.0, n, dtype=torch.float64)
    w = torch.exp(-0.5 * z * z) / math.sqrt(2 * math.pi)
    s = z * torch.sigmoid(z)
    return float(1.0 / math.sqrt(torch.trapezoid(s * s * w, z)))


SILU_GAIN = _silu_gain()


class ScalarMLPFunction(torch.nn.Module):
    def __init__(
        self,
        input_dim: int,
        output_dim: int,
        hidden_layers_depth: int = 0,
        hidden_layers_width: Optional[int] = None,
        nonlinearity: Optional[str] = "silu",
        bias: bool = False,
        forward_weight_init: bool = True,
    ):
        super().__init__()
        if bias:
            raise NotImplementedError("bias=True is not used by Allegro models (allegro_models.py:204-210)")
        if nonlinearity not in ("silu", None):
            raise NotImplementedError(f"nonlinearity {nonlinearity!r}: only 'silu' / None have CUDA kernels")
        if hidden_layers_depth > 0 and hidden_layers_width is None:
            raise ValueError("hidden_layers_width required")
        self.dims = [input_dim] + hidden_layers_depth * [hidden_layers_width] + [output_dim]
        self.nonlinearity = nonlinearity
        self.is_nonlinear = hidden_layers_depth > 0 and nonlinearity is not None
        self.weights = torch.nn.ParameterList()
        self.alphas: List[float] = []
        gain = 1.0
        for h_in, h_out in zip(self.dims, self.dims[1:]):
            w = torch.empty(h_in, h_out)
            torch.nn.init.uniform_(w, -math.sqrt(3), math.sqrt(3))
            self.weights.append(torch.nn.Parameter(w))
            self.alphas.append(gain / math.sqrt(h_in if forward_weight_init else h_out))
            gain = SILU_GAIN if nonlinearity == "silu" else 1.0

    @property
    def input_dim(self):
        return self.dims[0]

    @property
    def output_dim(self):
        return self.dims[-1]

    def folded_weights(self) -> List[torch.Tensor]:
        return [a * w.detach().double() for w, a in zip(self.weights, self.alphas)]

    def forward(self, x: torch.Tensor) -> torch.Tensor:
        n = len(self.weights)
        for k, (w, a) in enumerate(zip(self.weights, self.alphas)):
            x = x @ (a * w).to(x.dtype)
            if k < n - 1 and self.nonlinearity == "silu":
                x = torch.nn.functional.silu(x)
        return x


class PackedMLP:

    def __init__(self, mlp: ScalarMLPFunction, dtype: torch.dtype, device, out_perm=None, in_perm=None, extra_first=None, post=None):
        ws = [w.cpu() for w in mlp.folded_weights()]
        if extra_first is not None:
            extra_first = [w.detach().double().cpu() for w in extra_first]
        if post is not None:
            post = post.detach().double().cpu()
        if extra_first is not None:
            assert len(ws) == 1
            ws = [torch.cat([ws[0]] + list(extra_first), dim=1)]
        if in_perm is not None:
            ws[0] = ws[0][in_perm, :]
        if out_perm is not None:
            ws[-1] = ws[-1][:, out_perm]
        if post is not None:
            ws[-1] = ws[-1].to(torch.float64) @ post.to(torch.float64)
        self.W64 = [w.detach().to(torch.float64).cpu() for w in ws]
        self.silu = mlp.nonlinearity == "silu"
        self.W = [w.to(device=device, dtype=dtype).contiguous() for w in ws]
        self.WT = [w.T.to(device=device, dtype=dtype).contiguous() for w in ws]
        self.Wp = [_lib.linear_pack(w) for w in self.W]
        self.WTp = [_lib.linear_pack(w) for w in self.WT]
        self.out_pad = None
        n_out = ws[-1].shape[1]
        if n_out < 16 and dtype != torch.float64:
            wt = torch.zeros(16, ws[-1].shape[0], dtype=torch.float64)
            wt[:n_out] = ws[-1].T
            self.out_pad = wt.to(device=device, dtype=dtype).contiguous()
            self.out_pad_p = _lib.linear_pack(self.out_pad)
        self.dims = [ws[0].shape[0]] + [w.shape[1] for w in ws]
        self.dtype = dtype
        self.device = device

    @property
    def n_layers(self):
        return len(self.W)

    def forward(self, in_segs: Sequence[torch.Tensor], out_segs: Sequence[torch.Tensor]) -> List[torch.Tensor]:
        M = in_segs[0].shape[0]
        pre: List[torch.Tensor] = []
        cur = list(in_segs)
        for k in range(self.n_layers):
            last = k == self.n_layers - 1
            act = _lib.ACT_SILU if (k > 0 and self.silu) else _lib.ACT_NONE
            if last:
                _lib.linear(cur, self.W[k], out_segs, act=act, W_packed=self.Wp[k])
            else:
                h = torch.empty(M, self.dims[k + 1], dtype=self.dtype, device=self.device)
                _lib.linear(cur, self.W[k], [h], act=act, W_packed=self.Wp[k])
                pre.append(h)
                cur = [h]
        return pre

    def backward(self, gout_segs: Sequence[torch.Tensor], pre: List[torch.Tensor], gin_segs: Sequence[torch.Tensor], gin_accum: Sequence[bool]):
        M = gout_segs[0].shape[0]
        cur = list(gout_segs)
        WT, WTp = list(self.WT), list(self.WTp)
        if self.out_pad is not None and self.out_pad_p is not None and len(cur) == 1 and cur[0].is_contiguous():
            pad = torch.zeros(M, 16, dtype=self.dtype, device=self.device)
            pad[:, : cur[0].shape[1]] = cur[0]
            cur = [pad]
            WT[-1], WTp[-1] = self.out_pad, self.out_pad_p
        for k in range(self.n_layers - 1, -1, -1):
            if k == 0:
                _lib.linear(cur, WT[0], gin_segs, o_accum=gin_accum, W_packed=WTp[0])
            else:
                g = torch.empty(M, self.dims[k], dtype=self.dtype, device=self.device)
                if self.silu:
                    _lib.linear(cur, WT[k], [g], epi=_lib.EPI_MUL_DSILU, aux=pre[k - 1], W_packed=WTp[k])
                else:
                    _lib.linear(cur, WT[k], [g], W_packed=WTp[k])
                cur = [g]

    @property
    def is_two_layer_silu(self) -> bool:
        return self.n_layers == 2 and self.silu

    def hidden_grad(self, gout_segs: Sequence[torch.Tensor]) -> torch.Tensor:
        M = gout_segs[0].shape[0]
        g_h = torch.empty(M, self.dims[1], dtype=self.dtype, device=self.device)
        _lib.linear(list(gout_segs), self.WT[1], [g_h], W_packed=self.WTp[1])
        return g_h

    def backward_plain(self, gout_segs: Sequence[torch.Tensor], pre: List[torch.Tensor], gin_segs: Sequence[torch.Tensor]):
        g_h = self.hidden_grad(gout_segs)
        _lib.linear([g_h], self.WT[0], list(gin_segs), act=_lib.ACT_MUL_DSILU, a_aux=[pre[0]], W_packed=self.WTp[0])
```

### include/allegro_b200.h

```cpp
#ifndef ALLEGRO_B200_H
#define ALLEGRO_B200_H
#include <stdint.h>

#ifdef __cplusplus
extern "C" {
#endif

enum { AB2_F64 = 0, AB2_F32 = 1, AB2_BF16 = 2 };
enum { AB2_ACT_NONE = 0, AB2_ACT_SILU = 1, AB2_ACT_MUL_DSILU = 2 };
enum { AB2_EPI_NONE = 0, AB2_EPI_MUL_DSILU = 1 };

#define AB2_MAX_SEG 4
#define AB2_MAX_LMAX 4

const char* ab2_last_error(void);
int ab2_version(void);
int ab2_device_ok(void);
int ab2_set_option(const char* key, int value);


int ab2_op_scatter_env(int dtype, int64_t E, int64_t row , double sf,
                       const void* x2, const int64_t* idxs, void* gamma, void* stream);

int ab2_op_contract(int dtype, int mode, int64_t E, int U, int d1, int d2, int dout, int nnz,
                    const int32_t* tab_ijk, const void* cgw, const void* a, const void* b,
                    const int64_t* idxs, void* out, void* stream);

int ab2_op_contract_wgrad(int dtype, int64_t E, int U, int d1, int d2, int dout, int nnz,
                          const int32_t* tab_ijk, const void* x1, const void* gamma, const void* gout,
                          const int64_t* idxs, void* gcgw, void* stream);

int ab2_op_gather_rows(int dtype, int64_t E, int64_t row, double sf, const void* src,
                       const int64_t* idxs, void* out, void* stream);


int ab2_sh_fwd(int acc_dtype, int lmax, int64_t E, const void* vec, void* Y, void* stream);
int ab2_sh_bwd(int acc_dtype, int lmax, int64_t E, const void* vec, const void* gY, void* gvec,
               int accumulate, void* stream);

int ab2_linear(int dtype, int64_t M, int K, int N, int n_a, const void* const* a_ptr_host,
               const int64_t* a_ld_host, const int32_t* a_width_host,
               const void* const* a_aux_ptr_host , const int64_t* a_aux_ld_host,
               int act, const void* W,
               const void* W_packed ,
               int n_o, void* const* o_ptr_host, const int64_t* o_ld_host,
               const int32_t* o_width_host, const int32_t* o_accum_host, int epi, const void* aux,
               int64_t aux_ld, void* stream);

int64_t ab2_linear_packed_bytes(int dtype, int K, int N);
int ab2_linear_pack(int dtype, int K, int N, const void* W, void* packed, void* stream);

int ab2_env_sum(int dtype, int lmax, int64_t N, int U, const int32_t* row_ptr, const void* Y,
                const void* w, int64_t w_ld, double sf, void* gamma, void* stream);

int ab2_env_bwd(int dtype, int lmax, int64_t N, int64_t E, int U, const int32_t* row_ptr,
                const int32_t* ctr, const void* Y, const void* w, int64_t w_ld, const void* ggamma,
                double sf, void* gw, int64_t gw_ld, void* gY, void* stream);

int ab2_tp_fwd(int dtype, int lmax, int64_t N, int64_t E, int U, int d_in, int d_out, int nnz,
               const int32_t* tab_ijk, const void* cgw, const int32_t* row_ptr, const int32_t* ctr,
               const void* gamma, const void* Vin, int implicit_v0, const void* Y, const void* w0,
               int64_t w0_ld, void* Vout, void* stream);

int ab2_tp_bwd(int dtype, int lmax, int64_t N, int64_t E, int U, int d_in, int d_out, int nnz,
               const int32_t* tab_ijk, const void* cgw, const int32_t* row_ptr, const int32_t* ctr,
               const void* gamma, const void* Vin, int implicit_v0, const void* Y, const void* w0,
               int64_t w0_ld, const void* gVout, void* gVin, void* gw0, int64_t gw0_ld, void* gY,
               void* ggamma, void* stream);

int ab2_edge_sum(int acc_dtype, int64_t N, const int32_t* row_ptr, const void* Ez, double factor,
                 void* Ei, void* stream);
int ab2_edge_sum_bwd(int acc_dtype, int64_t E, const int32_t* ctr, const void* gEi, double factor,
                     void* gEz, void* stream);

int ab2_force_scatter(int acc_dtype, int64_t N, int64_t n_total, int64_t E, const int32_t* row_ptr,
                      const int32_t* col_ptr, const int32_t* col_perm, const void* gvec, void* F,
                      void* stream);


int ab2_edge_vec(int pos_dtype, int acc_dtype, int64_t E, const void* pos, const int32_t* ctr,
                 const int32_t* nbr, const void* shift, void* vec, void* stream);

int ab2_radial_fwd(int dtype, int64_t E, int S_rc, int num_bessels, double p_cut, const void* vec,
                   const int32_t* ctr, const int32_t* nbr, const int32_t* types,
                   const void* rmax_table, int num_types, const void* bessel_w, const void* Wb,
                   const void* center_embed, const void* neighbor_embed, void* e0, void* stream);
int ab2_radial_bwd(int dtype, int64_t E, int S_rc, int num_bessels, double p_cut, const void* vec,
                   const int32_t* ctr, const int32_t* nbr, const int32_t* types,
                   const void* rmax_table, int num_types, const void* bessel_w, const void* Wb,
                   const void* center_embed, const void* neighbor_embed, const void* g_e0,
                   void* gvec, void* stream);


int ab2_nl_bin(int pos_dtype, int64_t n, const void* pos, const double* box_host, const double* origin_host,
               const int32_t* pbc_host, const int32_t* ncell_host, double r_max, int32_t* cell_id, void* stream);
int ab2_nl_count(int pos_dtype, int64_t n_centres, const void* pos, const double* box_host,
                 const double* origin_host, const int32_t* pbc_host, const int32_t* ncell_host, double r_max,
                 const int32_t* cell_start, const int32_t* order, int32_t* counts, void* stream);
int ab2_nl_fill(int pos_dtype, int64_t n_centres, const void* pos, const double* box_host,
                const double* origin_host, const int32_t* pbc_host, const int32_t* ncell_host, double r_max,
                const int32_t* cell_start, const int32_t* order, const int32_t* row_ptr, int32_t* nbr,
                void* shift, void* stream);

int ab2_radial_pq_fwd(int dtype, int64_t E, int S, int num_bessels, double p_cut, const void* vec,
                      const int32_t* ctr, const int32_t* nbr, const int32_t* types, const void* rmax_table,
                      int num_types, const void* bessel_w, const void* PQ, void* out, void* stream);
int ab2_radial_pq_bwd(int dtype, int64_t E, int S, int num_bessels, double p_cut, const void* vec,
                      const int32_t* ctr, const int32_t* nbr, const int32_t* types, const void* rmax_table,
                      int num_types, const void* bessel_w, const void* PQ, const void* g_out, const void* aux,
                      void* gvec, void* stream);

int ab2_zbl(int acc_dtype, int64_t E, int num_types, double p_cut, double qq, const void* vec, const int32_t* ctr,
            const int32_t* nbr, const int32_t* types, const void* Z, const void* rmax_table, void* Ez, void* gvec,
            void* stream);


int64_t ab2_p2p_mailbox_bytes(int max_rows, int world);
int ab2_p2p_alloc(int64_t bytes, void** ptr);
int ab2_p2p_free(void* ptr);
int ab2_p2p_get_handle(void* ptr, void* handle64_host);
int ab2_p2p_open_handle(const void* handle64_host, void** ptr);
int ab2_p2p_close_handle(void* ptr);
int ab2_p2p_error(void* my_mailbox, int max_rows, int world, void* stream);
int ab2_p2p_begin(void* step_counter, void* stream);
int ab2_p2p_push_rows(int src_dtype, int kind, int side, const void* src, const int64_t* idx, int n, double shift_x,
                      void* peer_mailbox, int max_rows, int world, const void* step_counter, void* done_counter,
                      void* stream);
int ab2_p2p_wait_unpack(int dst_dtype, int kind, int side, void* my_mailbox, int max_rows, int world,
                        const void* step_counter, int n, void* dst, const int64_t* idx, int accumulate, void* stream);
int ab2_p2p_allreduce_energy(const void* e_local, int rank, int world, int max_rows, void* const* peers_dev,
                             void* my_mailbox, const void* step_counter, void* e_total, void* stream);

int ab2_transpose_ui(int dtype, int64_t E, int U, int d, const void* src, void* dst, int to_internal,
                     void* stream);

#ifdef __cplusplus
}
#endif
#endif
```

Baseline: 4.379 million.

## Fold readout MLP's second layer into first-layer GEMM epilogues

For a two-layer SiLU MLP with a scalar output, the forward pass now computes the first GEMM and folds SiLU plus the dot with the second-layer weights into the tensor-core epilogue as a per-row reduction. The backward pass becomes a single GEMM against a precomputed W1·diag(w2) matrix, with a dSiLU prologue and a per-row gradient-scale epilogue. This removes a second GEMM launch and its intermediate traffic in both directions. It adds new epilogue modes, an env toggle, and slice accumulation of row_out across N-slices. The fallback path uses an extra rowdot kernel, and the backward path no longer multiplies by a separate hidden gradient.

```diff
diff --git a/allegro_b200/_lib.py b/allegro_b200/_lib.py
--- a/allegro_b200/_lib.py
+++ b/allegro_b200/_lib.py
@@ -9,8 +9,8 @@
 from . import build as _build
 
 AB2_F64, AB2_F32, AB2_BF16 = 0, 1, 2
-ACT_NONE, ACT_SILU, ACT_MUL_DSILU = 0, 1, 2
-EPI_NONE, EPI_MUL_DSILU = 0, 1
+ACT_NONE, ACT_SILU, ACT_MUL_DSILU, ACT_DSILU = 0, 1, 2, 3
+EPI_NONE, EPI_MUL_DSILU, EPI_ROW_SCALE, EPI_SILU_ROWDOT = 0, 1, 2, 3
 MAX_SEG = 4
 
 DTYPE_ENUM = {torch.float64: AB2_F64, torch.float32: AB2_F32, torch.bfloat16: AB2_BF16}
@@ -32,6 +32,7 @@
     "ab2_sh_fwd": ([_i32, _i32, _i64, _vp, _vp, _vp], C.c_int),
     "ab2_sh_bwd": ([_i32, _i32, _i64, _vp, _vp, _vp, _i32, _vp], C.c_int),
     "ab2_linear": ([_i32, _i64, _i32, _i32, _i32, _vp, _vp, _vp, _vp, _vp, _i32, _vp, _vp, _i32, _vp, _vp, _vp, _vp, _i32, _vp, _i64, _vp], C.c_int),
+    "ab2_linear_ex": ([_i32, _i64, _i32, _i32, _i32, _vp, _vp, _vp, _vp, _vp, _i32, _vp, _vp, _i32, _vp, _vp, _vp, _vp, _i32, _vp, _i64, _vp, _vp], C.c_int),
     "ab2_linear_packed_bytes": ([_i32, _i32, _i32], C.c_int64),
     "ab2_linear_pack": ([_i32, _i32, _i32, _vp, _vp, _vp], C.c_int),
     "ab2_env_sum": ([_i32, _i32, _i64, _i32, _vp, _vp, _vp, _i64, _dbl, _vp, _vp], C.c_int),
@@ -205,6 +206,7 @@
     aux: Optional[torch.Tensor] = None,
     W_packed: Optional[torch.Tensor] = None,
     a_aux: Optional[Sequence[Optional[torch.Tensor]]] = None,
+    row_out: Optional[torch.Tensor] = None,
 ):
     M = a_segs[0].shape[0]
     K, N = W.shape
@@ -245,11 +247,18 @@
     if aux is not None:
         aux, aux_ld = _row_strided(aux, "aux")
         assert aux.dtype == dt
+        if epi == EPI_ROW_SCALE:
+            assert aux.shape[0] == M
+        elif epi == EPI_SILU_ROWDOT:
+            assert aux.numel() == N and aux.is_contiguous()
+    if epi == EPI_SILU_ROWDOT:
+        assert row_out is not None and row_out.dtype == dt and row_out.numel() == M
+        _contig(row_out, "row_out")
     with _timed("linear", 1):
         _check(
-            load().ab2_linear(
+            load().ab2_linear_ex(
                 DTYPE_ENUM[dt], M, K, N, na, a_ptr, a_ld, a_w, x_ptr, x_ld, act, _ptr(_contig(W, "W")), _ptr(W_packed), no, o_ptr, o_ld, o_w, o_acc, epi,
-                _ptr(aux), aux_ld, _stream(),
+                _ptr(aux), aux_ld, _ptr(row_out), _stream(),
             )
         )
 
diff --git a/allegro_b200/csrc/linear.cu b/allegro_b200/csrc/linear.cu
--- a/allegro_b200/csrc/linear.cu
+++ b/allegro_b200/csrc/linear.cu
@@ -66,6 +66,7 @@
             if (m < p.M && k0 + kk < p.K) {
                 v = lin_load_a<TAct, TAcc>(p, m, k0 + kk);
                 if (p.act == AB2_ACT_SILU) v = silu_f(v);
+                else if (p.act == AB2_ACT_DSILU) v = dsilu_f(v);
             }
             As[kk][r] = v;
         }
@@ -103,6 +104,7 @@
             if (n >= p.N) continue;
             TAcc v = acc[i][j];
             if (p.epi == AB2_EPI_MUL_DSILU) v *= dsilu_f(to_acc<TAcc>(((const TAct*)p.aux)[m * p.aux_ld + n]));
+            else if (p.epi == AB2_EPI_ROW_SCALE) v *= to_acc<TAcc>(((const TAct*)p.aux)[m * p.aux_ld]);
 #pragma unroll
             for (int s = 0; s < AB2_MAX_SEG; ++s) {
                 if (s < p.n_o) {
@@ -119,19 +121,35 @@
     }
 }
 
+template <typename TAct, typename TAcc>
+__global__ void __launch_bounds__(256) silu_rowdot_kernel(int64_t M, int N, const TAct* __restrict__ out, int64_t ld,
+                                                          const TAct* __restrict__ w, TAct* __restrict__ row_out) {
+    const int64_t m = ((int64_t)blockIdx.x * blockDim.x + threadIdx.x) >> 5;
+    const int lane = threadIdx.x & 31;
+    if (m >= M) return;
+    TAcc s = TAcc(0);
+    for (int n = lane; n < N; n += 32) s += silu_f(to_acc<TAcc>(out[m * ld + n])) * to_acc<TAcc>(w[n]);
+#pragma unroll
+    for (int o = 16; o > 0; o >>= 1) s += __shfl_xor_sync(0xffffffffu, s, o);
+    if (lane == 0) row_out[m] = from_acc<TAct>(s);
+}
+
 int ab2_linear_tc_try(int dtype, int64_t M, int K, int N, int n_a, const void* const* a_ptr, const int64_t* a_ld,
                       const int32_t* a_width, const void* const* a_aux, const int64_t* a_aux_ld, int act, const void* Wpacked, int n_o, void* const* o_ptr, const int64_t* o_ld,
-                      const int32_t* o_width, const int32_t* o_accum, int epi, const void* aux, int64_t aux_ld, cudaStream_t st);
-
-extern "C" int ab2_linear(int dtype, int64_t M, int K, int N, int n_a, const void* const* a_ptr, const int64_t* a_ld,
-                          const int32_t* a_width, const void* const* a_aux, const int64_t* a_aux_ld, int act, const void* W,
-                          const void* Wpacked, int n_o, void* const* o_ptr,
-                          const int64_t* o_ld, const int32_t* o_width, const int32_t* o_accum, int epi, const void* aux,
-                          int64_t aux_ld, void* stream) {
+                      const int32_t* o_width, const int32_t* o_accum, int epi, const void* aux, int64_t aux_ld, void* row_out, cudaStream_t st);
+
+extern "C" int ab2_linear_ex(int dtype, int64_t M, int K, int N, int n_a, const void* const* a_ptr, const int64_t* a_ld,
+                             const int32_t* a_width, const void* const* a_aux, const int64_t* a_aux_ld, int act, const void* W,
+                             const void* Wpacked, int n_o, void* const* o_ptr,
+                             const int64_t* o_ld, const int32_t* o_width, const int32_t* o_accum, int epi, const void* aux,
+                             int64_t aux_ld, void* row_out, void* stream) {
     if (M == 0) return 0;
     AB2_CHECK_ARG(n_a >= 1 && n_a <= AB2_MAX_SEG && n_o >= 1 && n_o <= AB2_MAX_SEG, "segment count");
     AB2_CHECK_ARG(K > 0 && N > 0 && W, "shape");
-    AB2_CHECK_ARG(epi == AB2_EPI_NONE || aux, "aux required for dsilu epilogue");
+    AB2_CHECK_ARG(epi == AB2_EPI_NONE || aux, "aux required for the epilogue");
+    AB2_CHECK_ARG(act >= AB2_ACT_NONE && act <= AB2_ACT_DSILU && epi >= AB2_EPI_NONE && epi <= AB2_EPI_SILU_ROWDOT, "act / epi mode");
+    AB2_CHECK_ARG(epi != AB2_EPI_SILU_ROWDOT || (row_out && n_o == 1 && !(o_accum && o_accum[0])),
+                  "silu row-dot epilogue: row_out, one output segment, no accumulation");
     LinParams p;
     memset(&p, 0, sizeof(p));
     p.M = M; p.K = K; p.N = N; p.n_a = n_a; p.act = act; p.W = W; p.n_o = n_o; p.epi = epi; p.aux = aux; p.aux_ld = aux_ld;
@@ -151,7 +169,7 @@
     AB2_CHECK_ARG(ns == N, "output segment widths must sum to N");
     cudaStream_t st = (cudaStream_t)stream;
     const int tc = Wpacked ? ab2_linear_tc_try(dtype, M, K, N, n_a, a_ptr, a_ld, a_width, a_aux, a_aux_ld, act, Wpacked, n_o, o_ptr, o_ld, o_width,
-                                               o_accum, epi, aux, aux_ld, st)
+                                               o_accum, epi, aux, aux_ld, row_out, st)
                            : -1;
     if (tc == 0) {
         AB2_CUDA_LAUNCH_CHECK();
@@ -164,5 +182,19 @@
     dim3 grid(ab2_blocks(M, 64), (unsigned)((N + 63) / 64));
     AB2_DISPATCH_DTYPE(dtype, linear_kernel<TAct, TAcc><<<grid, 256, 0, st>>>(p));
     AB2_CUDA_LAUNCH_CHECK();
+    if (epi == AB2_EPI_SILU_ROWDOT) {
+        AB2_DISPATCH_DTYPE(dtype, (silu_rowdot_kernel<TAct, TAcc><<<ab2_blocks(M, 8), 256, 0, st>>>(
+                                      M, N, (const TAct*)o_ptr[0], o_ld[0], (const TAct*)aux, (TAct*)row_out)));
+        AB2_CUDA_LAUNCH_CHECK();
+    }
     return 0;
 }
+
+extern "C" int ab2_linear(int dtype, int64_t M, int K, int N, int n_a, const void* const* a_ptr, const int64_t* a_ld,
+                          const int32_t* a_width, const void* const* a_aux, const int64_t* a_aux_ld, int act, const void* W,
+                          const void* Wpacked, int n_o, void* const* o_ptr,
+                          const int64_t* o_ld, const int32_t* o_width, const int32_t* o_accum, int epi, const void* aux,
+                          int64_t aux_ld, void* stream) {
+    return ab2_linear_ex(dtype, M, K, N, n_a, a_ptr, a_ld, a_width, a_aux, a_aux_ld, act, W, Wpacked, n_o, o_ptr, o_ld, o_width, o_accum, epi,
+                         aux, aux_ld, nullptr, stream);
+}
diff --git a/allegro_b200/csrc/linear_tc.cu b/allegro_b200/csrc/linear_tc.cu
--- a/allegro_b200/csrc/linear_tc.cu
+++ b/allegro_b200/csrc/linear_tc.cu
@@ -53,6 +53,8 @@
     int pf_mode;
     int raw_depth;
     int has_aux;
+    void* row_out;
+    int row_accum;
 };
 
 struct KEnt {
@@ -343,7 +345,7 @@
         auto row_of = [&](int itr) { const int r = itr * 4 + rsub; return full ? r : (r < rows_left ? r : rows_left - 1); };
         float* pfw = sPf + q * 2 * 32 * EPI_LD;
         auto prefetch = [&](int c0) {
-            if constexpr (PF == 0) return;
+            if constexpr (PF == 0 || PF == 3) return;
             if (c0 < p.Npad && rows_left > 0) {
                 const ChunkInfo ci = sChunk[c0 >> 5];
                 if (ci.ok && (PF == 1 || ci.accum)) {
@@ -360,9 +362,13 @@
         };
         prefetch(0);
         prefetch(32);
+        const int64_t m = tile * BM + q * 32 + lane;
+        float rscale = 0.f;
+        if constexpr (PF == 3)
+            if (p.epi == AB2_EPI_ROW_SCALE && m < p.M) rscale = to_acc<float>(((const TSrc*)p.aux)[m * p.aux_ld]);
+        float rdot = 0.f;
         mbar_wait(tfull_bar(a), aphase);
         tc_fence_after();
-        const int64_t m = tile * BM + q * 32 + lane;
         const uint32_t t_row = tmem_base + ((uint32_t)(q * 32) << 16) + (uint32_t)(a * 256);
         auto process = [&](int c0, const uint32_t (&r)[16]) {
             if (m >= p.M) return;
@@ -427,8 +433,24 @@
             tmem_ld16_nowait(t_row + c0, r0);
             if (two) tmem_ld16_nowait(t_row + c0 + 16, r1);
             tmem_ld_wait();
+            if constexpr (PF != 3) {
+            } else if (p.epi == AB2_EPI_ROW_SCALE) {
+#pragma unroll
+                for (int j = 0; j < 16; ++j) {
+                    r0[j] = __float_as_uint(__uint_as_float(r0[j]) * rscale);
+                    r1[j] = __float_as_uint(__uint_as_float(r1[j]) * rscale);
+                }
+            } else if (p.epi == AB2_EPI_SILU_ROWDOT) {
+                const TSrc* w = (const TSrc*)p.aux + c0;
+#pragma unroll
+                for (int j = 0; j < 16; ++j) {
+                    if (c0 + j < p.N) rdot += silu_fast(to_acc<float>(from_acc<TSrc>(__uint_as_float(r0[j])))) * to_acc<float>(w[j]);
+                    if (two && c0 + 16 + j < p.N)
+                        rdot += silu_fast(to_acc<float>(from_acc<TSrc>(__uint_as_float(r1[j])))) * to_acc<float>(w[16 + j]);
+                }
+            }
             const ChunkInfo ci = sChunk[c0 >> 5];
-            if constexpr (PF != 0) cp_async_wait<1>();
+            if constexpr (PF == 1 || PF == 2) cp_async_wait<1>();
             if ((p.debug & 1) || rows_left == 0) {
             } else if (ci.ok) {
                 float4* srow = reinterpret_cast<float4*>(stg + lane * EPI_LD);
@@ -485,7 +507,7 @@
                 process(c0, r0);
                 if (two) process(c0 + 16, r1);
             }
-            if constexpr (PF != 0) {
+            if constexpr (PF == 1 || PF == 2) {
                 __syncwarp();
                 prefetch(c0 + 64);
             }
@@ -493,6 +515,12 @@
         tc_fence_before();
         if (p.debug & 8) mbar_arrive(tempty_bar(a));
         else mbar_arrive_relaxed(tempty_bar(a));
+        if constexpr (PF == 3) {
+            if (p.epi == AB2_EPI_SILU_ROWDOT && m < p.M) {
+                TSrc* ro = (TSrc*)p.row_out + m;
+                *ro = from_acc<TSrc>(p.row_accum ? to_acc<float>(*ro) + rdot : rdot);
+            }
+        }
     }
 }
 
@@ -509,7 +537,7 @@
     const int raw_stage = RAW_STAGE * (p.has_aux ? 2 : 1);
     float* sEpi = reinterpret_cast<float*>(sRaw + p.raw_depth * raw_stage);
     float* sPf = reinterpret_cast<float*>(reinterpret_cast<uint8_t*>(sEpi) + EPI_BYTES);
-    uint64_t* bars = reinterpret_cast<uint64_t*>(reinterpret_cast<uint8_t*>(sEpi) + EPI_BYTES + (PF ? PF_BYTES : 0));
+    uint64_t* bars = reinterpret_cast<uint64_t*>(reinterpret_cast<uint8_t*>(sEpi) + EPI_BYTES + ((PF == 1 || PF == 2) ? PF_BYTES : 0));
     uint32_t* tmem_slot = reinterpret_cast<uint32_t*>(bars + 2 * NSTAGE + 4);
     static_assert((2 * NSTAGE + 4) * 8 == TAIL_BARS, "barrier block size");
     ChunkInfo* sChunk = reinterpret_cast<ChunkInfo*>(reinterpret_cast<uint8_t*>(bars) + TAIL_BARS + TAIL_SLOT);
@@ -671,6 +699,9 @@
                 if (p.act == AB2_ACT_SILU) {
 #pragma unroll
                     for (int t = 0; t < 8; ++t) v[i][t] = silu_fast(v[i][t]);
+                } else if (p.act == AB2_ACT_DSILU) {
+#pragma unroll
+                    for (int t = 0; t < 8; ++t) v[i][t] = dsilu_fast(v[i][t]);
                 }
                 const int g = warp * GPW + i;
                 const uint32_t off = g * (KC / 8) * 128 + kc * 128 + r8 * 16;
@@ -750,7 +781,7 @@
     uint8_t* sA = sW + ((w_bytes + 127) & ~127);
     float* sEpi = reinterpret_cast<float*>(sA + p.nstage * stage_bytes);
     float* sPf = reinterpret_cast<float*>(reinterpret_cast<uint8_t*>(sEpi) + EPI_BYTES);
-    uint64_t* bars = reinterpret_cast<uint64_t*>(reinterpret_cast<uint8_t*>(sEpi) + EPI_BYTES + (PF ? PF_BYTES : 0));
+    uint64_t* bars = reinterpret_cast<uint64_t*>(reinterpret_cast<uint8_t*>(sEpi) + EPI_BYTES + ((PF == 1 || PF == 2) ? PF_BYTES : 0));
     uint32_t* tmem_slot = reinterpret_cast<uint32_t*>(bars + 2 * NSTAGE + 4);
     ChunkInfo* sChunk = reinterpret_cast<ChunkInfo*>(reinterpret_cast<uint8_t*>(bars) + TAIL_BARS + TAIL_SLOT);
     int4* sKseg = reinterpret_cast<int4*>(reinterpret_cast<uint8_t*>(sChunk) + TAIL_CHUNK);
@@ -872,6 +903,9 @@
                 if (p.act == AB2_ACT_SILU) {
 #pragma unroll
                     for (int t = 0; t < 8; ++t) v[i][t] = silu_fast(v[i][t]);
+                } else if (p.act == AB2_ACT_DSILU) {
+#pragma unroll
+                    for (int t = 0; t < 8; ++t) v[i][t] = dsilu_fast(v[i][t]);
                 }
                 const int g = sub * RGW + i;
                 const uint32_t off = g * (KC / 8) * 128 + kc * 128 + r8 * 16;
@@ -992,7 +1026,7 @@
     int G = 0, NR = 0, nstage = 0;
     size_t smem = 0;
     for (int q = 0; q < 6 && !G; ++q) {
-        const size_t need = 1024 + ((w_bytes + 127) & ~127) + (size_t)plans[q][2] * stage_bytes + EPI_BYTES + (pf_mode ? PF_BYTES : 0) + TAIL_BYTES +
+        const size_t need = 1024 + ((w_bytes + 127) & ~127) + (size_t)plans[q][2] * stage_bytes + EPI_BYTES + ((pf_mode == 1 || pf_mode == 2) ? PF_BYTES : 0) + TAIL_BYTES +
                             (size_t)plans[q][1] * raw_slot;
         if (need <= (size_t)max_smem) { G = plans[q][0]; NR = plans[q][1]; nstage = plans[q][2]; smem = need; }
     }
@@ -1010,20 +1044,23 @@
     if (G == 4) {
         if (pf_mode == 1) return go(linear_tma_kernel<1, 4>);
         if (pf_mode == 2) return go(linear_tma_kernel<2, 4>);
+        if (pf_mode == 3) return go(linear_tma_kernel<3, 4>);
         return go(linear_tma_kernel<0, 4>);
     }
     if (pf_mode == 1) return go(linear_tma_kernel<1, 2>);
     if (pf_mode == 2) return go(linear_tma_kernel<2, 2>);
+    if (pf_mode == 3) return go(linear_tma_kernel<3, 2>);
     return go(linear_tma_kernel<0, 2>);
 }
 
 static int tc_launch_slice(int dtype, int64_t M, int K, int N, int n_a, const void* const* a_ptr, const int64_t* a_ld,
                            const int32_t* a_width, const void* const* a_aux, const int64_t* a_aux_ld, int act, const void* Whi, const void* Wlo,
                            int n_o, void* const* o_ptr, const int64_t* o_ld, const int32_t* o_width, const int32_t* o_accum, int epi,
-                           const void* aux, int64_t aux_ld, cudaStream_t st, bool dry = false) {
+                           const void* aux, int64_t aux_ld, void* row_out, int row_accum, cudaStream_t st, bool dry = false) {
     const int has_aux = (act == AB2_ACT_MUL_DSILU && a_aux) ? 1 : 0;
     int pf_mode = 0;
-    if (dtype == AB2_F32) {
+    if (epi == AB2_EPI_ROW_SCALE || epi == AB2_EPI_SILU_ROWDOT) pf_mode = 3;
+    else if (dtype == AB2_F32) {
         if (epi == AB2_EPI_MUL_DSILU) pf_mode = 1;
         else if (o_accum) for (int s = 0; s < n_o; ++s) if (o_accum[s]) pf_mode = 2;
     }
@@ -1038,7 +1075,7 @@
     TcParams p;
     memset(&p, 0, sizeof(p));
     p.M = M; p.K = K; p.N = N; p.Npad = tc_npad(N); p.n_a = n_a; p.act = act; p.Wpacked = Whi; p.Wlo = Wlo; p.n_o = n_o;
-    p.epi = epi; p.aux = aux; p.aux_ld = aux_ld; p.num_tiles = (M + BM - 1) / BM;
+    p.epi = epi; p.aux = aux; p.aux_ld = aux_ld; p.row_out = row_out; p.row_accum = row_accum; p.num_tiles = (M + BM - 1) / BM;
     for (int s = 0; s < n_a; ++s) {
         p.a[s].ptr = a_ptr[s]; p.a[s].ld = a_ld[s]; p.a[s].width = a_width[s];
         p.a[s].aux = has_aux ? a_aux[s] : nullptr; p.a[s].aux_ld = has_aux ? a_aux_ld[s] : 0;
@@ -1054,7 +1091,7 @@
     const int plans[4][2] = {{4, NSTAGE}, {4, 2}, {2, NSTAGE}, {2, 2}};
     for (int q = 0; q < 4 && !nstage; ++q) {
         const size_t need = ((w_bytes + 127) & ~127) + (size_t)plans[q][1] * stage_bytes + (size_t)plans[q][0] * raw_stage + EPI_BYTES +
-                            (pf_mode ? PF_BYTES : 0) + TAIL_BYTES;
+                            ((pf_mode == 1 || pf_mode == 2) ? PF_BYTES : 0) + TAIL_BYTES;
         if ((int)need <= max_smem) { raw_depth = plans[q][0]; nstage = plans[q][1]; smem = need; }
     }
     if (!nstage) return -1;
@@ -1081,14 +1118,16 @@
     if (split) {
         if (pf_mode == 1) return go(linear_tc_kernel<float, true, 1>);
         if (pf_mode == 2) return go(linear_tc_kernel<float, true, 2>);
+        if (pf_mode == 3) return go(linear_tc_kernel<float, true, 3>);
         return go(linear_tc_kernel<float, true, 0>);
     }
+    if (pf_mode == 3) return go(linear_tc_kernel<bf16, false, 3>);
     return go(linear_tc_kernel<bf16, false, 0>);
 }
 
 int ab2_linear_tc_try(int dtype, int64_t M, int K, int N, int n_a, const void* const* a_ptr, const int64_t* a_ld,
                       const int32_t* a_width, const void* const* a_aux, const int64_t* a_aux_ld, int act, const void* Wpacked, int n_o, void* const* o_ptr, const int64_t* o_ld,
-                      const int32_t* o_width, const int32_t* o_accum, int epi, const void* aux, int64_t aux_ld, cudaStream_t st) {
+                      const int32_t* o_width, const int32_t* o_accum, int epi, const void* aux, int64_t aux_ld, void* row_out, cudaStream_t st) {
     if (!g_ab2_opt_linear_tc || !Wpacked || dtype == AB2_F64) return -1;
     if (ab2_linear_packed_bytes(dtype, K, N) == 0) return -1;
     const int esz = (dtype == AB2_F32) ? 4 : 2;
@@ -1109,7 +1148,7 @@
     while (true) {
         const int probe = width < N ? width : N;
         if (tc_launch_slice(dtype, M, K, probe, n_a, a_ptr, a_ld, a_width, a_aux, a_aux_ld, act, Wpacked, Wpacked, 1, o_ptr, o_ld, &probe, &any_accum, epi,
-                            aux, aux_ld, st, true) == 0)
+                            aux, aux_ld, row_out, 0, st, true) == 0)
             break;
         if (width <= 32) return -1;
         width = (width / 2 + 31) / 32 * 32;
@@ -1134,9 +1173,9 @@
             }
             seg_lo = seg_hi;
         }
-        const void* aux_s = aux ? reinterpret_cast<const uint8_t*>(aux) + (size_t)n0 * esz : nullptr;
+        const void* aux_s = (aux && epi != AB2_EPI_ROW_SCALE) ? reinterpret_cast<const uint8_t*>(aux) + (size_t)n0 * esz : aux;
         const int rc = tc_launch_slice(dtype, M, K, ns, n_a, a_ptr, a_ld, a_width, a_aux, a_aux_ld, act, hi + (size_t)n0 * K * 2,
-                                       lo + (size_t)n0 * K * 2, cnt, so_ptr, so_ld, so_w, so_acc, epi, aux_s, aux_ld, st);
+                                       lo + (size_t)n0 * K * 2, cnt, so_ptr, so_ld, so_w, so_acc, epi, aux_s, aux_ld, row_out, n0 > 0, st);
         if (rc != 0) return n0 == 0 ? -1 : 1;
     }
     return 0;
diff --git a/allegro_b200/nn/_mlp.py b/allegro_b200/nn/_mlp.py
--- a/allegro_b200/nn/_mlp.py
+++ b/allegro_b200/nn/_mlp.py
@@ -1,6 +1,7 @@
 from __future__ import annotations
 
 import math
+import os
 from typing import List, Optional, Sequence
 
 import torch
@@ -102,6 +103,13 @@
         self.dims = [ws[0].shape[0]] + [w.shape[1] for w in ws]
         self.dtype = dtype
         self.device = device
+        self.fold_w2 = None
+        if (self.n_layers == 2 and self.silu and n_out == 1 and self.Wp[0] is not None
+                and os.environ.get("ALLEGRO_B200_READOUT_FOLD", "1") == "1"):
+            w1, w2 = self.W64
+            self.fold_w2 = w2.T.to(device=device, dtype=dtype).contiguous()
+            self.fold_gW = (w1 * w2[:, 0]).T.to(device=device, dtype=dtype).contiguous()
+            self.fold_gWp = _lib.linear_pack(self.fold_gW)
 
     @property
     def n_layers(self):
@@ -109,6 +117,10 @@
 
     def forward(self, in_segs: Sequence[torch.Tensor], out_segs: Sequence[torch.Tensor]) -> List[torch.Tensor]:
         M = in_segs[0].shape[0]
+        if self.fold_w2 is not None and len(out_segs) == 1:
+            h = torch.empty(M, self.dims[1], dtype=self.dtype, device=self.device)
+            _lib.linear(list(in_segs), self.W[0], [h], epi=_lib.EPI_SILU_ROWDOT, aux=self.fold_w2, row_out=out_segs[0], W_packed=self.Wp[0])
+            return [h]
         pre: List[torch.Tensor] = []
         cur = list(in_segs)
         for k in range(self.n_layers):
@@ -125,6 +137,14 @@
 
     def backward(self, gout_segs: Sequence[torch.Tensor], pre: List[torch.Tensor], gin_segs: Sequence[torch.Tensor], gin_accum: Sequence[bool]):
         M = gout_segs[0].shape[0]
+        if self.fold_w2 is not None and len(gout_segs) == 1:
+            _lib.linear([pre[0]], self.fold_gW, list(gin_segs), o_accum=gin_accum, act=_lib.ACT_DSILU, epi=_lib.EPI_ROW_SCALE,
+                        aux=gout_segs[0], W_packed=self.fold_gWp)
+            return
+        if self.is_two_layer_silu and self.WTp[1] is not None and self.WTp[0] is not None and self.WTp[0].numel() <= 64 * 1024:
+            g_h = self.hidden_grad(gout_segs)
+            _lib.linear([g_h], self.WT[0], list(gin_segs), o_accum=gin_accum, act=_lib.ACT_MUL_DSILU, a_aux=[pre[0]], W_packed=self.WTp[0])
+            return
         cur = list(gout_segs)
         WT, WTp = list(self.WT), list(self.WTp)
         if self.out_pad is not None and self.out_pad_p is not None and len(cur) == 1 and cur[0].is_contiguous():
diff --git a/include/allegro_b200.h b/include/allegro_b200.h
--- a/include/allegro_b200.h
+++ b/include/allegro_b200.h
@@ -7,8 +7,8 @@
 #endif
 
 enum { AB2_F64 = 0, AB2_F32 = 1, AB2_BF16 = 2 };
-enum { AB2_ACT_NONE = 0, AB2_ACT_SILU = 1, AB2_ACT_MUL_DSILU = 2 };
-enum { AB2_EPI_NONE = 0, AB2_EPI_MUL_DSILU = 1 };
+enum { AB2_ACT_NONE = 0, AB2_ACT_SILU = 1, AB2_ACT_MUL_DSILU = 2, AB2_ACT_DSILU = 3 };
+enum { AB2_EPI_NONE = 0, AB2_EPI_MUL_DSILU = 1, AB2_EPI_ROW_SCALE = 2, AB2_EPI_SILU_ROWDOT = 3 };
 
 #define AB2_MAX_SEG 4
 #define AB2_MAX_LMAX 4
@@ -46,6 +46,12 @@
                int n_o, void* const* o_ptr_host, const int64_t* o_ld_host,
                const int32_t* o_width_host, const int32_t* o_accum_host, int epi, const void* aux,
                int64_t aux_ld, void* stream);
+int ab2_linear_ex(int dtype, int64_t M, int K, int N, int n_a, const void* const* a_ptr_host,
+                  const int64_t* a_ld_host, const int32_t* a_width_host,
+                  const void* const* a_aux_ptr_host, const int64_t* a_aux_ld_host, int act, const void* W,
+                  const void* W_packed, int n_o, void* const* o_ptr_host, const int64_t* o_ld_host,
+                  const int32_t* o_width_host, const int32_t* o_accum_host, int epi, const void* aux,
+                  int64_t aux_ld, void* row_out , void* stream);
 
 int64_t ab2_linear_packed_bytes(int dtype, int K, int N);
 int ab2_linear_pack(int dtype, int K, int N, const void* W, void* packed, void* stream);
```

After: 4.731 million, median of 6. +8.0%, better.
